# lambdaclass/noir_backend_using_gnark

Hardware: AMD Instinct MI355X
Metric: Groth16 prove ms + BN254 G1 MSM scalar-muls/sec at 2^20 / 2^24 constraints (higher is better)
Workload: dtype u32; 1 GPU; groth16_prove_bn254_synthetic_r1cs_2^20; constraints=1048576, wires=1048576, n_public=8, scalars=uniform, per_gpu_constraints=1048576, window_tables=True, parallelism=single GPU

## Files before the change

include/zkmi.h:

```cpp
#ifndef ZKMI_H
#define ZKMI_H
#include <stddef.h>
#include <stdint.h>
#ifdef __cplusplus
extern "C" {
#endif

typedef struct { uint64_t l[4]; } zk_fr;
typedef struct { uint64_t l[4]; } zk_fp;
typedef struct { zk_fp x, y; } zk_g1_affine;
typedef struct { zk_fp x0, x1, y0, y1; } zk_g2_affine;

typedef enum {
    ZK_OK = 0,
    ZK_ERR_LEN = -1,
    ZK_ERR_NB_TASKS = -2,
    ZK_ERR_NO_DEVICE = -3,
    ZK_ERR_HIP = -4,
    ZK_ERR_ARG = -5,
    ZK_ERR_HANDLE = -6,
    ZK_ERR_BUSY = -7
} zk_status;

typedef struct {
// ... 155 lines not shown
        const void *const *vks, const size_t *vk_lens, size_t n_keys, int vk_is_hex,
        const zk_g2_affine srs_g2[2], const uint32_t *key_of ,
        const zk_fr *public_inputs, size_t pub_stride,
        uint8_t *accepted, size_t *n_accepted);
int zk_bn254_plonk_verify_batch_keys_dev(const void *d_proofs, size_t proof_stride, size_t n_proofs,
        const void *const *vks, const size_t *vk_lens, size_t n_keys, int vk_is_hex,
        const zk_g2_affine srs_g2[2], const uint32_t *key_of ,
        const void *d_public_inputs, size_t pub_stride,
        uint8_t *accepted, size_t *n_accepted);

int zk_bn254_groth16_msm5_dev(const void *d_a, const void *d_b, const void *d_b2, const void *d_w, size_t nw,
                              const void *d_k, const void *d_wk, size_t nk, const void *d_z, const void *d_h, size_t nz,
                              uint64_t out_xyzz[96], void *stream);
int zk_bn254_groth16_msm5_pk(uint64_t pk_handle, const void *d_w, const void *d_h, uint64_t out_xyzz[96], void *stream);
int zk_bn254_groth16_msm5_pk_begin(uint64_t pk_handle, const void *d_w, uint64_t *session);
int zk_bn254_groth16_msm5_pk_end(uint64_t session, const void *d_h, uint64_t out_xyzz[96], void *stream);
int zk_bn254_groth16_msm5_pk_abort(uint64_t session);
int zk_bn254_groth16_msm5_session_stream(uint64_t session, void **stream_out);
int zk_bn254_groth16_finalize(uint64_t pk_handle, const uint64_t *partials, size_t n_partials, const zk_fr *r,
                              const zk_fr *s, uint8_t proof_out[128]);
int zk_bn254_groth16_finalize_batch(uint64_t pk_handle, const uint64_t *partials, size_t n_partials, const zk_fr *r, const zk_fr *s,
                                    size_t n_proofs, uint8_t *proofs_out);
int zk_bn254_groth16_finalize_batch_dev(uint64_t pk_handle, const void *d_partials, size_t n_partials, const void *d_r, const void *d_s,
                                        size_t n_proofs, void *d_proofs_out, void *stream);

typedef struct {
    size_t n_public, n_constraints, n_vars;
    const void *ql, *qr, *qo, *qm, *qk;
    const uint32_t *xa, *xb, *xc;
    int coeffs_on_device;
    int reserved;
} zk_plonk_circuit;
typedef struct {
    uint32_t log_n;
    size_t n_public, n_constraints, n_vars;
    const zk_fr *ql, *qr, *qm, *qo, *cqk, *lqk, *s1, *s2, *s3;
    const int64_t *permutation;
    const uint32_t *xa, *xb, *xc;
    const zk_g1_affine *vk_s , *vk_ql, *vk_qr, *vk_qm, *vk_qo, *vk_qk;
} zk_plonk_pk;
typedef struct {
    uint64_t size, n_public;
    zk_fr size_inv, generator, coset_shift;
    zk_g1_affine s[3], ql, qr, qm, qo, qk;
} zk_plonk_vk;
int zk_bn254_plonk_setup(const zk_plonk_circuit *circuit, uint64_t srs_handle, uint64_t *pk_handle, zk_plonk_vk *vk_out);
int zk_bn254_plonk_pk_load(const zk_plonk_pk *pk, uint64_t srs_handle, uint64_t *pk_handle);
int zk_bn254_plonk_pk_free(uint64_t pk_handle);
int zk_bn254_plonk_pk_lagrange_srs(uint64_t pk_handle);
int zk_bn254_plonk_pk_read(const void *data, size_t len, int is_hex, size_t n_vars, size_t n_constraints, const uint32_t *xa,
                           const uint32_t *xb, const uint32_t *xc, uint64_t srs_handle, uint64_t *pk_handle);
int zk_bn254_plonk_pk_write(uint64_t pk_handle, int as_hex, void *out, size_t cap, size_t *out_len);
int zk_bn254_plonk_pk_info(uint64_t pk_handle, size_t *domain_size, size_t *n_public, size_t *n_constraints, size_t *n_vars);
int zk_bn254_plonk_pk_export(uint64_t pk_handle, int which, zk_fr *out_host, size_t n);
enum { ZK_PLONK_PROOF_BYTES = 548 };
int zk_bn254_plonk_prove(uint64_t pk_handle, const void *solution, size_t n_vars, int on_device, const zk_fr blinders[9],
                         const zk_fr *challenges, uint8_t proof_out[ZK_PLONK_PROOF_BYTES]);
int zk_bn254_plonk_synth_qk_dev(void *d_qk, const void *d_ql, const void *d_qr, const void *d_qo, const void *d_qm, const void *d_xa,
                                const void *d_xb, const void *d_xc, const void *d_solution, size_t n_constraints, void *stream);

int zk_bn254_iop_sigma_dev(const void *d_perm, uint32_t log_n, void *d_sigma, void *stream);
int zk_bn254_iop_ratio_copy_batch_dev(const void *d_l, const void *d_r, const void *d_o, size_t in_stride, uint32_t log_n, size_t rows, const void *d_sigma,
                                      const void *d_beta, const void *d_gamma, void *d_z, size_t out_stride, void *stream);
int zk_bn254_iop_ratio_copy_batch(const zk_fr *l, const zk_fr *r, const zk_fr *o, uint32_t log_n, size_t rows, const uint32_t *perm, const zk_fr *beta,
                                  const zk_fr *gamma, zk_fr *z_out);
int zk_bn254_plonk_ratio_batch_dev(uint64_t pk_handle, const void *d_l, const void *d_r, const void *d_o, size_t in_stride, size_t rows, const void *d_beta,
                                   const void *d_gamma, void *d_z, size_t out_stride, void *stream);
int zk_bn254_fr_batch_invert_dev(void *d_a, size_t n, void *stream);

int zk_bn254_plonk_quotient_batch_dev(uint64_t pk_handle, const void *d_l, const void *d_r, const void *d_o, const void *d_z, size_t in_stride, const void *d_pub,
                                      size_t pub_stride, size_t rows, const void *d_alpha, const void *d_beta, const void *d_gamma, void *d_h, size_t out_stride,
                                      void *d_status, void *stream);

int zk_bn254_fr_poly_open_rows_dev(const void *d_f, size_t in_stride, size_t len, size_t rows, const void *d_points, void *d_q, size_t q_stride, void *d_values,
                                   void *stream);
int zk_bn254_plonk_linearize_batch_dev(uint64_t pk_handle, const void *d_l, const void *d_r, const void *d_o, const void *d_z, size_t in_stride, const void *d_h,
                                       size_t h_stride, size_t rows, const void *d_alpha, const void *d_beta, const void *d_gamma, const void *d_zeta, void *d_values,
                                       void *d_zquot, void *d_lin, void *d_fh, size_t out_stride, void *stream);
int zk_bn254_plonk_open_batch_dev(uint64_t pk_handle, const void *d_fh, const void *d_lin, const void *d_l, const void *d_r, const void *d_o, size_t in_stride,
                                  size_t rows, const void *d_zeta, const void *d_kzg_gamma, void *d_q, size_t out_stride, void *d_value, void *stream);
int zk_bn254_plonk_commit_batch_dev(uint64_t pk_handle, const void *d_rows, size_t row_stride, size_t len, size_t rows, int from_values, void *d_out,
                                    void *d_compressed);

int zk_bn254_plonk_prove_batch(uint64_t pk_handle, const void *solutions, size_t n_vars, size_t sol_stride, size_t rows, int on_device,
                               const zk_fr *blinders , const zk_fr *challenges , size_t chunk_rows ,
                               uint8_t *proofs_out , int *status_out );
int zk_bn254_plonk_prove_batch_info(uint64_t pk_handle, size_t *chunk_rows, int *commits_batched, int *lin_by_linearity);
int zk_bn254_plonk_challenges_batch_dev(uint64_t pk_handle, int stage, size_t rows, const void *d_pub, size_t pub_stride, const void *d_points,
                                        const void *d_prev, const void *d_values, void *d_out, void *stream);

enum { ZK_ACIR_LAYOUT_REFERENCE = 0, ZK_ACIR_LAYOUT_ONE_VAR_PER_WITNESS = 1 };
int zk_plonk_preprocess(const char *acir_json, size_t acir_len, const char *values_hex, size_t values_len, int layout,
                        uint64_t srs_handle, char *pk_hex_out, size_t pk_cap, size_t *pk_len, char *vk_hex_out, size_t vk_cap,
                        size_t *vk_len, uint64_t *pk_handle);
int zk_plonk_prove_with_pk(const char *acir_json, size_t acir_len, const char *values_hex, size_t values_len, int layout,
                           const char *pk_hex, size_t pk_len, uint64_t pk_handle, uint64_t srs_handle, const zk_fr *blinders,
                           char proof_hex_out[2 * ZK_PLONK_PROOF_BYTES]);
int zk_acir_to_sparse_r1cs(const char *acir_json, size_t acir_len, size_t n_values, int layout, size_t *n_public, size_t *n_vars,
                           size_t *n_constraints, zk_fr *ql, zk_fr *qr, zk_fr *qo, zk_fr *qm, zk_fr *qk, uint32_t *xa, uint32_t *xb,
                           uint32_t *xc, uint32_t *order);
int zk_acir_public_witnesses(const char *acir_json, size_t acir_len, size_t n_values, int layout, uint32_t *out, size_t cap, size_t *n_public);
int zk_export_cache_info(size_t *n_circuits, size_t *n_keys, size_t *bytes);
int zk_acir_lower_resident(const char *acir_json, size_t acir_len, size_t n_values, int layout, int with_coefficients);
int zk_export_cache_clear(void);
int zk_export_set_new_srs_size(size_t n);
size_t zk_export_new_srs_size(void);
int zk_bn254_plonk_pk_bytes(uint64_t handle, size_t *bytes);

int zk_groth16_r1cs_from_raw(const char *raw_json, size_t len, uint64_t *r1cs_handle, void **d_witness, size_t *n_wires, size_t *n_public);
int zk_groth16_preprocess(const char *raw_json, size_t raw_len, const zk_fr *toxic, char *pk_hex_out, size_t pk_cap, size_t *pk_len,
                          char *vk_hex_out, size_t vk_cap, size_t *vk_len, uint64_t *pk_handle);
int zk_groth16_prove_with_pk(const char *raw_json, size_t raw_len, const char *pk_hex, size_t pk_len, uint64_t pk_handle, const zk_fr *rs,
                             char proof_hex_out[256]);
int zk_groth16_prove_with_meta(const char *raw_json, size_t raw_len, const zk_fr *toxic, const zk_fr *rs, char proof_hex_out[256]);
int zk_groth16_lower_resident(const char *raw_json, size_t raw_len, int to_device);
int zk_groth16_key_resident(const char *pk_hex, size_t pk_len);
int zk_groth16_public_inputs(const char *raw_json, size_t raw_len, zk_fr *out, size_t cap, size_t *n_public);

enum {
    ZK_ROW_OK = 0,
    ZK_ROW_UNSATISFIED = 1,
    ZK_ROW_BAD_HEX = 2,
    ZK_ROW_NOT_CANONICAL = 3,
    ZK_ROW_BAD_COUNT = 4,
    ZK_ROW_BAD_PROOF_HEX
};
int zk_plonk_solutions_rows(const char *acir_json, size_t acir_len, int layout, const char *values_hex, size_t values_len, size_t values_stride,
                            size_t rows, void *d_solutions , size_t sol_stride, int *status_out );
int zk_groth16_wires_rows(const char *raw_json, size_t raw_len, const char *values_hex, size_t values_len, size_t values_stride,
                          size_t rows, void *d_wires , size_t wire_stride, int *status_out );
int zk_plonk_prove_batch_with_pk(const char *acir_json, size_t acir_len, int layout, const char *values_hex, size_t values_len, size_t values_stride,
                                 size_t rows, const char *pk_hex, size_t pk_len, uint64_t pk_handle, uint64_t srs_handle,
                                 const zk_fr *blinders , size_t chunk_rows ,
                                 char *proofs_hex_out , int *status_out );
int zk_groth16_prove_batch_with_pk(const char *raw_json, size_t raw_len, const char *values_hex, size_t values_len, size_t values_stride, size_t rows,
                                   const char *pk_hex, size_t pk_len, uint64_t pk_handle, const zk_fr *rs ,
                                   size_t chunk_rows, char *proofs_hex_out , int *status_out );

int zk_plonk_verify_batch_with_vk(const char *acir_json, size_t acir_len, int layout, const char *proofs_hex, size_t proofs_stride,
                                  const char *values_hex, size_t values_len, size_t values_stride, size_t rows, const char *vk_hex, size_t vk_len,
                                  const zk_g2_affine srs_g2[2], size_t chunk_rows, uint8_t *accepted , int *status_out ,
                                  size_t *n_accepted);
int zk_groth16_verify_batch_with_vk(const char *raw_json, size_t raw_len, const char *proofs_hex, size_t proofs_stride, const char *values_hex,
                                    size_t values_len, size_t values_stride, size_t rows, const char *vk_hex, size_t vk_len, size_t chunk_rows,
                                    uint8_t *accepted , int *status_out , size_t *n_accepted);

int zk_bn254_msm_plan_info(size_t n, int window_tables, uint32_t *window_bits, uint32_t *digits);

typedef struct {
    size_t n;
    int window_bits, scalars_mont, table, drop_zero_digits;
    uint32_t c, row_first, row_step, sets;
    size_t stride;
    int by_rows, reserved;
    const zk_fr *vec[3];
    size_t row_stride;
} zk_msm_prep_request;
typedef struct {
    uint32_t c, W, Wd, Wrows, B, nb, key_bits, L, Lmin, m1, N1, dropped;
    uint64_t total, max_tasks, device_total;
    uint32_t ctl[64];
    uint32_t *keys, *vals, *start, *task_off, *task_begin, *len_keys, *task_ids, *multi_list;
} zk_msm_prep_result;
int zk_bn254_msm_prep_inspect(const zk_msm_prep_request *req, zk_msm_prep_result *res);

#define ZK_MSM_TAIL_MAX_LEVELS 12
typedef struct {
    zk_msm_prep_request prep;
    const void *points;
    int is_g2, quad_tail, keep_final, reserved;
    uint32_t l1_m, l2_m, skip_below, reserved2;
} zk_msm_tail_request;
typedef struct {
    uint32_t kind, n_in, n_out, sh_in, sh_out, m;
} zk_msm_tail_level;
typedef struct {
    zk_msm_prep_result prep;
    uint32_t m2, tasks, n_final, sh_final, n_levels, reserved;
    zk_msm_tail_level level[ZK_MSM_TAIL_MAX_LEVELS];
    uint64_t table_entries, level_entries;
    uint64_t *table, *partial_acc, *partial_fold, *level_a, *level_s, *set_values, *total, *final_affine;
    uint8_t *final_bytes;
} zk_msm_tail_result;
int zk_bn254_msm_tail_inspect(const zk_msm_tail_request *req, zk_msm_tail_result *res);

#define ZK_HSCAN_ROWS_MAX 8
typedef struct {
    uint32_t rows, K, nb, pad;
    int eval_only, reserved;
    zk_fr *f[ZK_HSCAN_ROWS_MAX], *q[ZK_HSCAN_ROWS_MAX];
    size_t len[ZK_HSCAN_ROWS_MAX];
    zk_fr a[ZK_HSCAN_ROWS_MAX];
} zk_hscan_request;
typedef struct {
    uint32_t nb, reserved;
    zk_fr *tcarry, *btot_local, *btot, *total;
} zk_hscan_result;
int zk_bn254_hscan_inspect(const zk_hscan_request *req, zk_hscan_result *res);

int zk_bn254_felts_decode_hex(const char *hex, size_t hex_len, void *d_out, size_t cap, size_t *n_out);
int zk_bn254_felts_decode_hex_dev(const void *d_text, size_t text_len, void *d_out, size_t cap, size_t n, int to_mont,
                                  void *stream);
int zk_bn254_felts_decode_bytes_dev(const void *d_raw, size_t raw_len, void *d_out, size_t cap, size_t n, int to_mont,
                                    void *stream);
int zk_bn254_felts_encode_hex(const void *d_in, size_t n, char *hex_out, size_t cap);
int zk_bn254_felts_decode_hex_rows_dev(const void *d_text, size_t pitch, size_t rows, size_t n, void *d_out, size_t out_stride,
                                       int to_mont, int *d_status , void *stream);
int zk_bn254_bytes_decode_hex_rows_dev(const void *d_text, size_t pitch, size_t rows, size_t n_bytes, void *d_out, size_t out_stride,
                                       int *d_status , void *stream);
int zk_bn254_felts_public_hex_rows_dev(const void *d_text, size_t pitch, size_t rows, size_t n_values, const uint32_t *d_where, size_t n_public,
                                       void *d_pub, size_t pub_stride, int *d_status , void *stream);

int zk_bn254_fr_random_dev(void *d_out, size_t n, uint64_t seed, int mont, int witness_like, void *stream);
int zk_bn254_g1_generate_dev(void *d_out, size_t n, uint64_t seed, void *stream);
int zk_bn254_g2_generate_dev(void *d_out, size_t n, uint64_t seed, void *stream);
int zk_bn254_fr_mul_dev(void *d_out, const void *d_a, const void *d_b, size_t n, void *stream);

int zk_bn254_kzg_new_srs_dev(void *d_g1_out, size_t size, const zk_fr *alpha, zk_g2_affine g2_out[2], void *stream);
int zk_bn254_kzg_srs_read(const void *data, size_t len, int is_hex, int table_window_bits, uint64_t *handle, size_t *n_g1,
                          zk_g2_affine g2_out[2]);
int zk_bn254_kzg_srs_write(uint64_t handle, const zk_g2_affine g2[2], int as_hex, void *out, size_t cap, size_t *out_len);
int zk_bn254_kzg_srs_g2(const void *data, size_t len, int is_hex, zk_g2_affine g2_out[2]);

typedef struct { zk_g1_affine h; zk_fr claimed_value; } zk_kzg_opening;
int zk_bn254_kzg_open(uint64_t srs, const void *const *polys, const size_t *lens, const zk_fr *points, size_t count, int on_device, zk_kzg_opening *out);
int zk_bn254_kzg_batch_open_single_point(uint64_t srs, const void *const *polys, const size_t *lens, const zk_g1_affine *digests, size_t count,
                                         const zk_fr *point, int on_device, zk_g1_affine *out_h, zk_fr *out_claimed);
int zk_bn254_kzg_verify(const zk_g1_affine *digest, const zk_kzg_opening *opening, const zk_fr *point, const zk_g2_affine srs_g2[2], int *accepted);
int zk_bn254_kzg_fold_proof(const zk_g1_affine *digests, size_t count, const zk_g1_affine *h, const zk_fr *claimed, const zk_fr *point,
                            zk_kzg_opening *out_opening, zk_g1_affine *out_digest);
int zk_bn254_kzg_batch_verify_single_point(const zk_g1_affine *digests, size_t count, const zk_g1_affine *h, const zk_fr *claimed, const zk_fr *point,
                                           const zk_g2_affine srs_g2[2], int *accepted);
int zk_bn254_kzg_verify_batch(const zk_g1_affine *digests, const zk_kzg_opening *openings, const zk_fr *points, size_t n_openings,
                              const zk_g2_affine srs_g2[2], uint8_t *accepted, size_t *n_accepted);

int zk_dev_alloc(void **d_ptr, size_t bytes);
int zk_dev_free(void *d_ptr);
int zk_dev_h2d(void *d_dst, const void *h_src, size_t bytes);
int zk_dev_d2h(void *h_dst, const void *d_src, size_t bytes);
int zk_dev_sync(void);

int zk_profile_enable(int on);
int zk_profile_host(const char *name, double ms);
int zk_profile_reset(void);
int zk_profile_count(void);
int zk_profile_get(int idx, char *name_out, size_t name_cap, uint64_t *launches, double *total_ms);

int zk_selftest_host(void);

#ifdef __cplusplus
}
#endif
#endif
```

noir_backend_using_gnark_amd/_lib.py:

```python
from __future__ import annotations

import ctypes as C
import os

_HERE = os.path.dirname(os.path.abspath(__file__))
LIB_PATH = os.path.join(_HERE, "libzkmi.so")


def use_library(path: str) -> None:
    global LIB_PATH, _lib
    if _lib is not None:
        raise RuntimeError("the library is already loaded from %s" % LIB_PATH)
    LIB_PATH = path


ZK_OK, ZK_ERR_LEN, ZK_ERR_NB_TASKS, ZK_ERR_NO_DEVICE, ZK_ERR_HIP, ZK_ERR_ARG, ZK_ERR_HANDLE, ZK_ERR_BUSY = 0, -1, -2, -3, -4, -5, -6, -7


class ZkmiError(RuntimeError):
    def __init__(self, code: int, msg: str):
        super().__init__("libzkmi error %d: %s" % (code, msg))
        self.code = code


class MsmCfg(C.Structure):
    _fields_ = [("nb_tasks", C.c_int), ("scalars_mont", C.c_int), ("window_bits", C.c_int), ("device_mask", C.c_int)]


class MsmPrepRequest(C.Structure):
    _fields_ = [("n", C.c_size_t), ("window_bits", C.c_int), ("scalars_mont", C.c_int), ("table", C.c_int), ("drop_zero_digits", C.c_int),
                ("c", C.c_uint32), ("row_first", C.c_uint32), ("row_step", C.c_uint32), ("sets", C.c_uint32), ("stride", C.c_size_t),
                ("by_rows", C.c_int), ("reserved", C.c_int), ("vec", C.c_void_p * 3), ("row_stride", C.c_size_t)]


MSM_PREP_PLAN = ("c", "W", "Wd", "Wrows", "B", "nb", "key_bits", "L", "Lmin", "m1", "N1")
MSM_PREP_ARRAYS = ("keys", "vals", "start", "task_off", "task_begin", "len_keys", "task_ids", "multi_list")


class MsmPrepResult(C.Structure):
    _fields_ = [(k, C.c_uint32) for k in MSM_PREP_PLAN + ("dropped",)] + [("total", C.c_uint64), ("max_tasks", C.c_uint64), ("device_total", C.c_uint64),
                                                                         ("ctl", C.c_uint32 * 64)] + [(k, C.c_void_p) for k in MSM_PREP_ARRAYS]


MSM_TAIL_MAX_LEVELS = 12
MSM_TAIL_LEVEL = ("kind", "n_in", "n_out", "sh_in", "sh_out", "m")
MSM_TAIL_KINDS = {1: "l1", 2: "l2", 3: "wave", 4: "wave_quad"}
MSM_TAIL_ARRAYS = ("table", "partial_acc", "partial_fold", "level_a", "level_s", "set_values", "total", "final_affine", "final_bytes")


class MsmTailRequest(C.Structure):
    _fields_ = [("prep", MsmPrepRequest), ("points", C.c_void_p), ("is_g2", C.c_int), ("quad_tail", C.c_int), ("keep_final", C.c_int), ("reserved", C.c_int),
                ("l1_m", C.c_uint32), ("l2_m", C.c_uint32), ("skip_below", C.c_uint32), ("reserved2", C.c_uint32)]


class MsmTailLevel(C.Structure):
    _fields_ = [(k, C.c_uint32) for k in MSM_TAIL_LEVEL]


class MsmTailResult(C.Structure):
    _fields_ = [("prep", MsmPrepResult)] + [(k, C.c_uint32) for k in ("m2", "tasks", "n_final", "sh_final", "n_levels", "reserved")] + \
               [("level", MsmTailLevel * MSM_TAIL_MAX_LEVELS), ("table_entries", C.c_uint64), ("level_entries", C.c_uint64)] + \
               [(k, C.c_void_p) for k in MSM_TAIL_ARRAYS]


HSCAN_ROWS_MAX = 8


class HscanRequest(C.Structure):
    _fields_ = [("rows", C.c_uint32), ("K", C.c_uint32), ("nb", C.c_uint32), ("pad", C.c_uint32), ("eval_only", C.c_int), ("reserved", C.c_int),
                ("f", C.c_void_p * HSCAN_ROWS_MAX), ("q", C.c_void_p * HSCAN_ROWS_MAX), ("len", C.c_size_t * HSCAN_ROWS_MAX),
                ("a", (C.c_uint64 * 4) * HSCAN_ROWS_MAX)]


class HscanResult(C.Structure):
    _fields_ = [("nb", C.c_uint32), ("reserved", C.c_uint32)] + [(k, C.c_void_p) for k in ("tcarry", "btot_local", "btot", "total")]


class Groth16PK(C.Structure):
    _fields_ = [("log_domain", C.c_uint32), ("n_wires", C.c_size_t), ("n_public", C.c_size_t),
                ("g1_alpha", C.c_void_p), ("g1_beta", C.c_void_p), ("g1_delta", C.c_void_p),
                ("g1_a", C.c_void_p), ("g1_b", C.c_void_p), ("g1_k", C.c_void_p), ("g1_z", C.c_void_p),
                ("g2_beta", C.c_void_p), ("g2_delta", C.c_void_p), ("g2_b", C.c_void_p), ("bases_on_device", C.c_int), ("flags", C.c_int),
                ("infinity_a", C.c_void_p), ("infinity_b", C.c_void_p), ("nb_infinity_a", C.c_size_t), ("nb_infinity_b", C.c_size_t),
                ("table_window_bits", C.c_int), ("device_mask", C.c_int), ("shard_rank", C.c_uint32), ("shard_count", C.c_uint32)]


class R1CS(C.Structure):
    _fields_ = [("n_constraints", C.c_size_t), ("n_wires", C.c_size_t), ("n_public", C.c_size_t)] + \
               [(m + k, C.c_void_p) for m in ("l", "r", "o") for k in ("_ptr", "_idx", "_val")]


class PlonkCircuit(C.Structure):
    _fields_ = [("n_public", C.c_size_t), ("n_constraints", C.c_size_t), ("n_vars", C.c_size_t),
                ("ql", C.c_void_p), ("qr", C.c_void_p), ("qo", C.c_void_p), ("qm", C.c_void_p), ("qk", C.c_void_p),
                ("xa", C.c_void_p), ("xb", C.c_void_p), ("xc", C.c_void_p), ("coeffs_on_device", C.c_int), ("reserved", C.c_int)]


class PlonkPK(C.Structure):
    _fields_ = [("log_n", C.c_uint32), ("n_public", C.c_size_t), ("n_constraints", C.c_size_t), ("n_vars", C.c_size_t)] + \
               [(k, C.c_void_p) for k in ("ql", "qr", "qm", "qo", "cqk", "lqk", "s1", "s2", "s3", "permutation", "xa", "xb", "xc",
                                          "vk_s", "vk_ql", "vk_qr", "vk_qm", "vk_qo", "vk_qk")]


class PlonkVK(C.Structure):
    _fields_ = [("size", C.c_uint64), ("n_public", C.c_uint64), ("size_inv", C.c_uint64 * 4), ("generator", C.c_uint64 * 4), ("coset_shift", C.c_uint64 * 4),
                ("s", C.c_uint64 * 24), ("ql", C.c_uint64 * 8), ("qr", C.c_uint64 * 8), ("qm", C.c_uint64 * 8), ("qo", C.c_uint64 * 8), ("qk", C.c_uint64 * 8)]


PLONK_PROOF_BYTES = 548

SYMBOLS = [
    "zk_device_count", "zk_init", "zk_last_error", "zk_version",
    "zk_bn254_g1_msm", "zk_bn254_g2_msm", "zk_bn254_g1_msm_dev", "zk_bn254_g2_msm_dev",
    "zk_bn254_g1_msm_partial_dev", "zk_bn254_g2_msm_partial_dev", "zk_bn254_g1_sum_xyzz", "zk_bn254_g2_sum_xyzz",
    "zk_bn254_msm_plan_info", "zk_bn254_msm_prep_inspect", "zk_bn254_msm_tail_inspect", "zk_bn254_bases_register", "zk_bn254_bases_register_dev", "zk_bn254_bases_register_cfg", "zk_bn254_bases_build_table", "zk_bn254_bases_lagrange", "zk_bn254_bases_free", "zk_bn254_msm_bases", "zk_bn254_msm_bases_batch", "zk_bn254_msm_bases_batch_dev", "zk_bn254_msm_bases_dev", "zk_bn254_scalars_register", "zk_bn254_scalars_free", "zk_bn254_msm_bases_prepared",
    "zk_bn254_ntt", "zk_bn254_ntt_dev", "zk_bn254_bit_reverse", "zk_bn254_bit_reverse_dev",
    "zk_bn254_ntt_batch", "zk_bn254_ntt_batch_dev", "zk_bn254_groth16_compute_h_batch", "zk_bn254_groth16_compute_h_batch_dev",
    "zk_bn254_groth16_compute_h", "zk_bn254_groth16_compute_h_dev", "zk_bn254_groth16_h_shard_dev", "zk_bn254_ntt_shard_dev",
    "zk_bn254_felts_decode_hex", "zk_bn254_felts_decode_hex_dev", "zk_bn254_felts_decode_bytes_dev", "zk_bn254_felts_encode_hex",
    "zk_bn254_groth16_pk_load", "zk_bn254_groth16_pk_free", "zk_bn254_groth16_pk_info", "zk_bn254_groth16_prove",
    "zk_bn254_groth16_pk_read", "zk_bn254_groth16_pk_write", "zk_bn254_groth16_vk_write",
    "zk_bn254_groth16_verify", "zk_bn254_plonk_verify", "zk_bn254_pairing_check",
    "zk_bn254_pair", "zk_bn254_pair_host", "zk_bn254_groth16_verify_batch", "zk_bn254_plonk_verify_batch",
    "zk_bn254_r1cs_load", "zk_bn254_r1cs_free", "zk_bn254_r1cs_eval_abc_dev", "zk_bn254_r1cs_eval_abc_rows_dev", "zk_bn254_groth16_setup", "zk_bn254_groth16_prove_r1cs",
    "zk_bn254_groth16_prove_batch", "zk_bn254_groth16_prove_r1cs_batch", "zk_bn254_groth16_batch_info",
    "zk_bn254_groth16_msm5_dev", "zk_bn254_groth16_msm5_pk", "zk_bn254_groth16_msm5_pk_begin", "zk_bn254_groth16_msm5_pk_end", "zk_bn254_groth16_msm5_pk_abort", "zk_bn254_groth16_msm5_session_stream", "zk_bn254_groth16_finalize",
    "zk_bn254_groth16_finalize_batch", "zk_bn254_groth16_finalize_batch_dev",
    "zk_bn254_plonk_setup", "zk_bn254_plonk_pk_load", "zk_bn254_plonk_pk_free", "zk_bn254_plonk_pk_lagrange_srs", "zk_bn254_plonk_pk_export", "zk_bn254_plonk_pk_read", "zk_bn254_plonk_pk_write", "zk_bn254_plonk_prove", "zk_bn254_plonk_synth_qk_dev",
    "zk_bn254_iop_sigma_dev", "zk_bn254_iop_ratio_copy_batch_dev", "zk_bn254_iop_ratio_copy_batch", "zk_bn254_plonk_ratio_batch_dev", "zk_bn254_fr_batch_invert_dev", "zk_bn254_plonk_quotient_batch_dev",
    "zk_bn254_fr_poly_open_rows_dev", "zk_bn254_plonk_linearize_batch_dev", "zk_bn254_plonk_open_batch_dev",
    "zk_plonk_preprocess", "zk_plonk_prove_with_pk", "zk_bn254_plonk_pk_info", "zk_acir_to_sparse_r1cs", "zk_groth16_r1cs_from_raw",
    "zk_groth16_preprocess", "zk_groth16_prove_with_pk", "zk_groth16_prove_with_meta",
    "zk_bn254_fr_random_dev", "zk_bn254_g1_generate_dev", "zk_bn254_g2_generate_dev", "zk_bn254_fr_mul_dev", "zk_bn254_kzg_new_srs_dev", "zk_bn254_kzg_srs_read", "zk_bn254_kzg_srs_write",
    "zk_dev_alloc", "zk_dev_free", "zk_dev_h2d", "zk_dev_d2h", "zk_dev_sync",
    "zk_profile_enable", "zk_profile_reset", "zk_profile_count", "zk_profile_get", "zk_profile_host", "zk_selftest_host",
    "zk_init_devices", "zk_warm_streams", "zk_init_flags", "zk_bn254_kzg_srs_g2", "zk_device_entries", "zk_set_entry", "zk_set_default_devices", "zk_default_devices", "zk_bn254_ntt_devices",
    "zk_acir_public_witnesses", "zk_acir_lower_resident", "zk_export_cache_info", "zk_export_cache_clear", "zk_bn254_plonk_pk_bytes",
    "zk_groth16_lower_resident", "zk_groth16_key_resident", "zk_groth16_public_inputs", "zk_bn254_groth16_pk_build_tables", "zk_bn254_groth16_pk_bytes",
    "zk_export_set_new_srs_size", "zk_export_new_srs_size", "zk_warm_session_streams", "zk_warm_session_streams_background", "zk_background_wait", "zk_background_hold", "zk_background_set_yield_ms", "zk_bn254_bases_build_table_background",
    "zk_bn254_msm_bases_rows", "zk_bn254_msm_bases_rows_dev", "zk_bn254_msm_rows_info", "zk_bn254_plonk_commit_batch_dev",
    "zk_bn254_plonk_prove_batch", "zk_bn254_plonk_prove_batch_info", "zk_bn254_plonk_challenges_batch_dev",
    "zk_bn254_felts_decode_hex_rows_dev", "zk_plonk_solutions_rows", "zk_groth16_wires_rows", "zk_plonk_prove_batch_with_pk", "zk_groth16_prove_batch_with_pk",
    "zk_bn254_groth16_verify_batch_dev", "zk_bn254_plonk_verify_batch_dev", "zk_bn254_rows_sha256_dev", "zk_bn254_bytes_decode_hex_rows_dev",
    "zk_bn254_felts_public_hex_rows_dev", "zk_plonk_verify_batch_with_vk", "zk_groth16_verify_batch_with_vk",
    "zk_bn254_kzg_open", "zk_bn254_kzg_batch_open_single_point", "zk_bn254_kzg_verify", "zk_bn254_kzg_fold_proof", "zk_bn254_kzg_batch_verify_single_point", "zk_bn254_kzg_verify_batch",
    "zk_bn254_plonk_verify_batch_keys", "zk_bn254_plonk_verify_batch_keys_dev",
    "zk_bn254_hscan_inspect",
]

_SZ, _VP, _CP = C.c_size_t, C.c_void_p, C.c_char_p
ARGTYPES = {
    "zk_bn254_felts_decode_hex_rows_dev": [_VP, _SZ, _SZ, _SZ, _VP, _SZ, C.c_int, _VP, _VP],
    "zk_plonk_solutions_rows": [_CP, _SZ, C.c_int, _CP, _SZ, _SZ, _SZ, _VP, _SZ, _VP],
    "zk_groth16_wires_rows": [_CP, _SZ, _CP, _SZ, _SZ, _SZ, _VP, _SZ, _VP],
    "zk_plonk_prove_batch_with_pk": [_CP, _SZ, C.c_int, _CP, _SZ, _SZ, _SZ, _CP, _SZ, C.c_uint64, C.c_uint64, _VP, _SZ, _VP, _VP],
    "zk_groth16_prove_batch_with_pk": [_CP, _SZ, _CP, _SZ, _SZ, _SZ, _CP, _SZ, C.c_uint64, _VP, _SZ, _VP, _VP],
    "zk_bn254_groth16_verify_batch_dev": [_VP, _SZ, _SZ, _CP, _SZ, C.c_int, _VP, _SZ, _SZ, _VP, _VP],
    "zk_bn254_plonk_verify_batch_dev": [_VP, _SZ, _SZ, _CP, _SZ, C.c_int, _VP, _VP, _SZ, _SZ, _VP, _VP],
    "zk_bn254_rows_sha256_dev": [_VP, _SZ, _SZ, _VP, _SZ, _SZ, _SZ, _VP, _VP],
    "zk_bn254_bytes_decode_hex_rows_dev": [_VP, _SZ, _SZ, _SZ, _VP, _SZ, _VP, _VP],
    "zk_bn254_felts_public_hex_rows_dev": [_VP, _SZ, _SZ, _SZ, _VP, _SZ, _VP, _SZ, _VP, _VP],
    "zk_plonk_verify_batch_with_vk": [_CP, _SZ, C.c_int, _CP, _SZ, _CP, _SZ, _SZ, _SZ, _CP, _SZ, _VP, _SZ, _VP, _VP, _VP],
    "zk_groth16_verify_batch_with_vk": [_CP, _SZ, _CP, _SZ, _CP, _SZ, _SZ, _SZ, _CP, _SZ, _SZ, _VP, _VP, _VP],
    "zk_bn254_plonk_verify_batch_keys": [_VP, _SZ, _VP, _VP, _SZ, C.c_int, _VP, _VP, _VP, _SZ, _VP, _VP],
    "zk_bn254_plonk_verify_batch_keys_dev": [_VP, _SZ, _SZ, _VP, _VP, _SZ, C.c_int, _VP, _VP, _VP, _SZ, _VP, _VP],
}
ROW_OK, ROW_UNSATISFIED, ROW_BAD_HEX, ROW_NOT_CANONICAL, ROW_BAD_COUNT, ROW_BAD_PROOF_HEX = 0, 1, 2, 3, 4, 5

_lib = None


def lib() -> C.CDLL:
    global _lib
    if _lib is None:
        if not os.path.exists(LIB_PATH):
            raise RuntimeError(
                "libzkmi.so is missing at %s: build it with `python -c 'import __graft_entry__ as g; g.build()'` "
                "(make -C noir_backend_using_gnark_amd/csrc).  There is no CPU fallback for the product path." % LIB_PATH)
        _lib = C.CDLL(LIB_PATH)
        _lib.zk_last_error.restype = C.c_char_p
        _lib.zk_version.restype = C.c_char_p
        for name in SYMBOLS:
            fn = getattr(_lib, name)
            if name == "zk_export_new_srs_size":
                fn.restype = C.c_size_t
            elif name not in ("zk_last_error", "zk_version"):
                fn.restype = C.c_int
            if name in ARGTYPES:
                fn.argtypes = ARGTYPES[name]
    return _lib


def check(rc: int) -> None:
    if rc != ZK_OK:
# ... 81 lines not shown
```

noir_backend_using_gnark_amd/bn254.py:

```python
from __future__ import annotations

import ctypes as C
from dataclasses import dataclass

import numpy as np

from . import _lib
from ._lib import MsmCfg, check, lib, vp

DIT, DIF = 0, 1


@dataclass
class MultiExpConfig:
    nb_tasks: int = 0
    scalars_mont: bool = False
    window_bits: int = 0
    device_mask: int = 0

    def _c(self) -> MsmCfg:
        return MsmCfg(self.nb_tasks, 1 if self.scalars_mont else 0, self.window_bits, self.device_mask)


def _as_u64(a, width) -> np.ndarray:
    a = np.ascontiguousarray(a, dtype=np.uint64)
    if a.size % width:
        raise ValueError("array size %d is not a multiple of %d limbs" % (a.size, width))
    return a.reshape(-1, width)


def _multi_exp(fn, width, points, scalars, config):
    config = config or MultiExpConfig()
    points, scalars = _as_u64(points, width), _as_u64(scalars, 4)
    if points.shape[0] != scalars.shape[0]:
        pass
    out = np.zeros(width, dtype=np.uint64)
    cfg = config._c()
    rc = fn(vp(points), C.c_size_t(points.shape[0]), vp(scalars), C.c_size_t(scalars.shape[0]), C.byref(cfg), vp(out))
    if rc in (_lib.ZK_ERR_LEN, _lib.ZK_ERR_NB_TASKS):
        raise ValueError((lib().zk_last_error() or b"").decode())
    check(rc)
    return out


def g1_multi_exp(points, scalars, config: MultiExpConfig | None = None) -> np.ndarray:
    return _multi_exp(lib().zk_bn254_g1_msm, 8, points, scalars, config)


def g2_multi_exp(points, scalars, config: MultiExpConfig | None = None) -> np.ndarray:
    return _multi_exp(lib().zk_bn254_g2_msm, 16, points, scalars, config)


def g1_multi_exp_dev(d_points: int, d_scalars: int, n: int, config: MultiExpConfig | None = None, stream: int = 0, partial=False):
    cfg = (config or MultiExpConfig())._c()
    out = np.zeros(16 if partial else 8, dtype=np.uint64)
    fn = lib().zk_bn254_g1_msm_partial_dev if partial else lib().zk_bn254_g1_msm_dev
    check(fn(C.c_void_p(d_points), C.c_void_p(d_scalars), C.c_size_t(n), C.byref(cfg), vp(out), C.c_void_p(stream)))
    return out


def g2_multi_exp_dev(d_points: int, d_scalars: int, n: int, config: MultiExpConfig | None = None, stream: int = 0, partial=False):
    cfg = (config or MultiExpConfig())._c()
    out = np.zeros(32 if partial else 16, dtype=np.uint64)
    fn = lib().zk_bn254_g2_msm_partial_dev if partial else lib().zk_bn254_g2_msm_dev
    check(fn(C.c_void_p(d_points), C.c_void_p(d_scalars), C.c_size_t(n), C.byref(cfg), vp(out), C.c_void_p(stream)))
    return out


def g1_sum_partials(partials) -> np.ndarray:
    p = _as_u64(partials, 16)
    out = np.zeros(8, dtype=np.uint64)
    check(lib().zk_bn254_g1_sum_xyzz(vp(p), C.c_size_t(p.shape[0]), vp(out)))
    return out


def g2_sum_partials(partials) -> np.ndarray:
    p = _as_u64(partials, 32)
    out = np.zeros(16, dtype=np.uint64)
    check(lib().zk_bn254_g2_sum_xyzz(vp(p), C.c_size_t(p.shape[0]), vp(out)))
    return out


def _msm_prep_request(req, vectors, n, window_bits, scalars_mont, table_c, stride, row_first, row_step, rows, row_stride, drop_zero_digits):
    if rows:
        mat = _as_u64(vectors, 4)
        row_stride = row_stride if row_stride is not None else mat.shape[0] // rows
        if n is None:
            n = row_stride
        if mat.shape[0] < (rows - 1) * row_stride + n:
            raise ValueError("the matrix is shorter than rows * row_stride")
        keep, sets = [mat], rows
    else:
        keep, seen = [], {}
        for v in (vectors if isinstance(vectors, (list, tuple)) else [vectors]):
            if id(v) not in seen:
                seen[id(v)] = _as_u64(v, 4)
            keep.append(seen[id(v)])
        sets = len(keep)
        if n is None:
            n = keep[0].shape[0]
        if any(k.shape[0] < n for k in keep):
            raise ValueError("a scalar vector is shorter than n")
    req.n, req.window_bits, req.scalars_mont, req.table, req.drop_zero_digits = n, window_bits, int(scalars_mont), int(table_c != 0), int(drop_zero_digits)
    req.c, req.row_first, req.row_step, req.sets, req.stride = table_c, row_first, row_step, sets, (stride if stride is not None else n)
    req.by_rows, req.row_stride = int(rows > 0), (row_stride or 0)
    for i, k in enumerate(keep[:3]):
        req.vec[i] = k.ctypes.data
    return keep


def _msm_prep_plan(res) -> dict:
    return dict({k: int(getattr(res, k)) for k in _lib.MSM_PREP_PLAN}, total=int(res.total), max_tasks=int(res.max_tasks))


def _msm_prep_arrays(res, plan, arrays) -> dict:
    sizes = dict(keys=plan["total"], vals=plan["total"], start=plan["nb"] + 1, task_off=plan["nb"] + 1, task_begin=plan["max_tasks"], len_keys=plan["max_tasks"],
                 task_ids=plan["max_tasks"], multi_list=plan["nb"])
    wanted = _lib.MSM_PREP_ARRAYS if arrays is None else tuple(arrays)
    out = {k: np.zeros(sizes[k] if k in wanted else 0, np.uint32) for k in _lib.MSM_PREP_ARRAYS}
    for k in wanted:
        setattr(res, k, out[k].ctypes.data)
    return out


def msm_prep_inspect(vectors, n: int | None = None, window_bits: int = 0, scalars_mont: bool = False, table_c: int = 0, stride: int | None = None,
                     row_first: int = 0, row_step: int = 1, rows: int = 0, row_stride: int | None = None, drop_zero_digits: bool = False,
                     plan_only: bool = False, arrays=None) -> dict:
    req = _lib.MsmPrepRequest()
    keep = _msm_prep_request(req, vectors, n, window_bits, scalars_mont, table_c, stride, row_first, row_step, rows, row_stride, drop_zero_digits)
    res = _lib.MsmPrepResult()
    check(lib().zk_bn254_msm_prep_inspect(C.byref(req), C.byref(res)))
    out = _msm_prep_plan(res)
    if plan_only or out["total"] == 0:
        out.update(device_total=0, dropped=False, ctl=np.zeros(64, np.uint32), **{k: np.zeros(0, np.uint32) for k in _lib.MSM_PREP_ARRAYS})
        return out
    arrays = _msm_prep_arrays(res, out, arrays)
    check(lib().zk_bn254_msm_prep_inspect(C.byref(req), C.byref(res)))
    assert _msm_prep_plan(res) == out
    out.update(device_total=int(res.device_total), dropped=bool(res.dropped), ctl=np.array(res.ctl[:], dtype=np.uint32), **arrays)
    return out


def msm_tail_inspect(points, vectors, is_g2: bool = False, l1_m: int = 0, l2_m: int = 0, quad_tail: bool = False, keep_final: bool = False, skip_below: int = 0,
                     plan_only: bool = False, **prep) -> dict:
    width = 16 if is_g2 else 8
    pts = _as_u64(points, width)
    req = _lib.MsmTailRequest()
    keep = _msm_prep_request(req.prep, vectors, prep.pop("n", None), prep.pop("window_bits", 0), prep.pop("scalars_mont", False), prep.pop("table_c", 0),
                             prep.pop("stride", None), prep.pop("row_first", 0), prep.pop("row_step", 1), prep.pop("rows", 0), prep.pop("row_stride", None),
                             prep.pop("drop_zero_digits", False))
    if prep:
        raise TypeError("unknown arguments: %s" % sorted(prep))
    if pts.shape[0] < req.prep.n:
        raise ValueError("fewer points than scalars")
    req.points, req.is_g2, req.quad_tail, req.keep_final = pts.ctypes.data, int(is_g2), int(quad_tail), int(keep_final)
    req.l1_m, req.l2_m, req.skip_below = l1_m, l2_m, skip_below
    res = _lib.MsmTailResult()
    check(lib().zk_bn254_msm_tail_inspect(C.byref(req), C.byref(res)))

    def plan():
        d = _msm_prep_plan(res.prep)
        d.update({k: int(getattr(res, k)) for k in ("m2", "n_final", "sh_final", "table_entries", "level_entries")})
        d["levels"] = [dict({k: int(getattr(res.level[i], k)) for k in _lib.MSM_TAIL_LEVEL}, kind=_lib.MSM_TAIL_KINDS[int(res.level[i].kind)])
                       for i in range(res.n_levels)]
        return d
    out = plan()
    sets = int(req.prep.sets) if req.prep.table else 1
    if plan_only or (out["total"] == 0 and not keep_final):
        return out
    arrays = _msm_prep_arrays(res.prep, out, None) if out["total"] else {}
    W = out["W"]
    shapes = dict(table=(out["table_entries"], width), partial_acc=(out["max_tasks"], width), partial_fold=(out["max_tasks"], width),
                  level_a=(out["level_entries"], width), level_s=(out["level_entries"], width))
    if keep_final:
        shapes.update(final_affine=(sets, 8), final_bytes=(sets, 32))
    else:
        shapes.update(set_values=(W, width), total=(1, width))
    tail = {k: np.zeros(shp, np.uint8 if k == "final_bytes" else np.uint64) for k, shp in shapes.items()}
    for k, a in tail.items():
        setattr(res, k, a.ctypes.data)
    check(lib().zk_bn254_msm_tail_inspect(C.byref(req), C.byref(res)))
    assert plan() == out
    if out["total"]:
        out.update(device_total=int(res.prep.device_total), dropped=bool(res.prep.dropped), ctl=np.array(res.prep.ctl[:], dtype=np.uint32), **arrays)
    out["tasks"] = int(res.tasks)
    at = 0
    for lv in out["levels"]:
        cnt = W * lv["n_out"]
        lv["A"] = tail["level_a"][at:at + cnt].reshape(W, lv["n_out"], width)
        lv["S"] = tail["level_s"][at:at + cnt].reshape(W, lv["n_out"], width)
        at += cnt
    out.update({k: v for k, v in tail.items() if k not in ("level_a", "level_s")})
    return out


MSM_ROWS_SPARSE, MSM_ROWS_NO_POINTS = 1, 2
_DEV = (int, _lib.DeviceBuffer)


def _dptr(a) -> int:
    return a if isinstance(a, int) else a.ptr


def _check_len(rc: int) -> None:
    if rc in (_lib.ZK_ERR_LEN, _lib.ZK_ERR_NB_TASKS):
        raise ValueError((lib().zk_last_error() or b"").decode())
    check(rc)


def rows_digests(dev_call, host_call, scalars, n, rows, row_stride, out, compressed, points):
    if not isinstance(compressed, bool) and not isinstance(compressed, _DEV):
        raise TypeError("compressed must be False, True or a device buffer / pointer")
    if not points and compressed is False:
        raise ValueError("points=False leaves nothing to return: ask for the compressed digests")
    if not points and out is not None:
        raise ValueError("out takes the points: there are none with points=False")
    if isinstance(scalars, _DEV):
        if n is None or rows is None:
            raise ValueError("n and rows are required with device-resident scalars")
        n, rows = int(n), int(rows)
        if n < 0 or rows < 0:
            raise ValueError("n and rows must not be negative")
        row_stride = int(n if row_stride is None else row_stride)
        if row_stride < n and rows > 1:
            raise ValueError("row_stride = %d is below the n = %d scalars of a row" % (row_stride, n))
        span = ((rows - 1) * row_stride + n) * 32 if rows and n else 0
        if isinstance(scalars, _lib.DeviceBuffer) and span > scalars.nbytes:
            raise ValueError("scalars: %d bytes do not fit the device buffer (%d bytes)" % (span, scalars.nbytes))
        seen = [("scalars", scalars, span)]
        for name, b, nbytes in (("out", out, rows * 64), ("compressed", compressed, rows * 32)):
            if b is None or isinstance(b, bool):
                continue
            if not isinstance(b, _DEV):
                raise TypeError("%s must be a device buffer or a device pointer" % name)
            if isinstance(b, _lib.DeviceBuffer) and nbytes > b.nbytes:
                raise ValueError("%s: %d bytes do not fit the device buffer (%d bytes)" % (name, nbytes, b.nbytes))
            for other, c, cb in seen:
                if nbytes and cb and _dptr(b) < _dptr(c) + cb and _dptr(c) < _dptr(b) + nbytes:
                    raise ValueError("%s overlaps %s" % (name, other))
            seen.append((name, b, nbytes))
        made = []
        if points and out is None:
            out = _lib.DeviceBuffer(max(rows * 64, 64))
            made.append(out)
        if compressed is True:
            compressed = _lib.DeviceBuffer(max(rows * 32, 32))
            made.append(compressed)
        enc = None if compressed is False else compressed
        if rows:
            try:
                _check_len(dev_call(_dptr(scalars), row_stride, n, rows, _dptr(out) if points else 0, _dptr(enc) if enc is not None else 0))
            except Exception:
                for b in made:
                    b.free()
                raise
        return out if enc is None else ((out, enc) if points else enc)
    if not (isinstance(scalars, np.ndarray) and scalars.dtype == np.uint64 and scalars.flags["C_CONTIGUOUS"]):
        raise TypeError("scalars must be a C-contiguous uint64 numpy array (or a device buffer)")
    if scalars.ndim != 3 or scalars.shape[2] != 4:
        raise ValueError("scalars has shape %s, not (rows, n, 4)" % (scalars.shape,))
    cnt, width = scalars.shape[0], scalars.shape[1]
    for name, v, want in (("rows", rows, cnt), ("n", n, width), ("row_stride", row_stride, width)):
        if v is not None and int(v) != want:
            raise ValueError("%s = %d != %d of the host array (its rows are contiguous)" % (name, v, want))
    if out is not None or not isinstance(compressed, bool):
        raise ValueError("out and a compressed buffer belong to the device form: the host form returns new arrays")
    pts = np.zeros((cnt, 8), np.uint64) if points else None
    enc = np.zeros((cnt, 32), np.uint8) if compressed else None
    if cnt and host_call is not None:
        _check_len(host_call(scalars, width, cnt, pts, enc))
    elif cnt:
        bufs = [_lib.DeviceBuffer.from_numpy(scalars), _lib.DeviceBuffer(cnt * 64), _lib.DeviceBuffer(cnt * 32)]
        try:
            _check_len(dev_call(bufs[0].ptr, width, width, cnt, bufs[1].ptr if points else 0, bufs[2].ptr if compressed else 0))
            pts = bufs[1].to_numpy(np.uint64, (cnt, 8)) if points else None
            enc = bufs[2].to_numpy(np.uint8, (cnt, 32)) if compressed else None
        finally:
            for b in bufs:
                b.free()
    return pts if enc is None else ((pts, enc) if points else enc)


def msm_rows_info(bases: "ResidentBases", n: int, sparse: bool = False) -> dict:
    chunk, batched = C.c_size_t(0), C.c_int(0)
    _check_len(lib().zk_bn254_msm_rows_info(bases.handle, C.c_size_t(n), C.c_uint32(MSM_ROWS_SPARSE if sparse else 0), C.byref(chunk), C.byref(batched)))
    return {"chunk_rows": int(chunk.value), "batched": bool(batched.value)}


class ResidentBases:

    def __init__(self, points, is_g2: bool = False, n: int | None = None, table_window_bits: int = 0):
        self.is_g2, self.handle = is_g2, C.c_uint64(0)
        if isinstance(points, (_lib.DeviceBuffer, int)):
            if n is None:
                raise ValueError("n is required with device-resident points")
            self.n = n
            ptr = points.ptr if isinstance(points, _lib.DeviceBuffer) else int(points)
            check(lib().zk_bn254_bases_register_cfg(C.c_void_p(ptr), C.c_size_t(n), C.c_int(int(is_g2)), C.c_int(1), C.c_int(table_window_bits), C.byref(self.handle)))
            return
        points = _as_u64(points, 16 if is_g2 else 8)
        self.n = points.shape[0]
        check(lib().zk_bn254_bases_register_cfg(vp(points), C.c_size_t(self.n), C.c_int(int(is_g2)), C.c_int(0), C.c_int(table_window_bits), C.byref(self.handle)))

    def multi_exp_dev(self, d_scalars, n: int, config: MultiExpConfig | None = None, offset: int = 0) -> np.ndarray:
        out = np.zeros(16 if self.is_g2 else 8, dtype=np.uint64)
        cfg = (config or MultiExpConfig())._c()
        ptr = d_scalars.ptr if isinstance(d_scalars, _lib.DeviceBuffer) else int(d_scalars)
        rc = lib().zk_bn254_msm_bases_dev(self.handle, C.c_size_t(offset), C.c_void_p(ptr), C.c_size_t(n), C.byref(cfg), vp(out))
        if rc in (_lib.ZK_ERR_LEN, _lib.ZK_ERR_NB_TASKS):
            raise ValueError((lib().zk_last_error() or b"").decode())
        check(rc)
        return out

    def multi_exp(self, scalars, config: MultiExpConfig | None = None, offset: int = 0) -> np.ndarray:
# ... 213 lines not shown
```

noir_backend_using_gnark_amd/csrc/msm.hip:

```cpp
#include <math.h>
#include <string.h>

#include <algorithm>
#include <memory>
#include <tuple>
#include <type_traits>

#ifdef ZKMI_EXPERIMENTS
#include "experiments/msm_rocprim_include.inc"
#endif

#include <chrono>
#include "codec_dev.hpp"
#include "ctx.hpp"
#include "curve.hpp"
#include "ff29.hpp"
#include "host_ff.hpp"
#include "msm.hpp"
#include "multidev.hpp"
#include "proofio.hpp"
#include "radix.hpp"

namespace zkmi {

struct PingPong {
    uint32_t* b[2];
    int cur = 0;
    PingPong(uint32_t* x, uint32_t* y) : b{x, y} {}
    uint32_t* current() const { return b[cur]; }
    uint32_t* alternate() const { return b[cur ^ 1]; }
    void swap() { cur ^= 1; }
};
#ifdef ZKMI_EXPERIMENTS
#include "experiments/msm_rocprim_config.inc"
#endif

static int rs_sort_pairs(Slot* s, hipStream_t st, void* tmp, PingPong& kb, PingPong& vb, size_t n, unsigned key_bits, const uint32_t* d_n = nullptr) {
    const RsPlan R = rs_plan(n, key_bits);
    uint32_t* tile_hist = (uint32_t*)tmp;
    uint32_t* ghist = tile_hist + (size_t)RS_MAX_BINS * R.ntiles;
    uint32_t* gbase = ghist + RS_MAX_PASSES * RS_MAX_BINS;
    RsArgs A;
    A.npass = R.npass;
    for (unsigned p = 0; p < RS_MAX_PASSES; p++) { A.shift[p] = R.shift[p]; A.bits[p] = R.bits[p]; }
    const unsigned nt = (unsigned)R.ntiles;
    ZK_HIP(hipMemsetAsync(ghist, 0, RS_MAX_PASSES * RS_MAX_BINS * 4, st));
    ZK_LAUNCH(s, st, "msm_sort_hist", k_rs_hist, dim3(nt), dim3(RS_THREADS), 0, (const uint32_t*)kb.current(), (uint32_t)n, A, nt, ghist, tile_hist, d_n);
    ZK_LAUNCH(s, st, "msm_sort_bases", k_rs_bases, dim3(1), dim3(RS_MAX_BINS), 0, (const uint32_t*)ghist, gbase, R.npass);
    for (unsigned p = 0; p < R.npass; p++) {
        if (p) ZK_LAUNCH(s, st, "msm_sort_hist", k_rs_tile_hist, dim3(nt), dim3(RS_THREADS), 0, (const uint32_t*)kb.current(), (uint32_t)n, R.shift[p], R.bits[p], nt, tile_hist, d_n);
        ZK_LAUNCH(s, st, "msm_sort_scan", k_rs_scan_rows, dim3(1u << R.bits[p]), dim3(256), 0, tile_hist, nt);
        ZK_LAUNCH(s, st, "msm_sort_pass", k_rs_scatter, dim3(nt), dim3(RS_THREADS), 0, (const uint32_t*)kb.current(), (const uint32_t*)vb.current(), kb.alternate(), vb.alternate(),
                  (uint32_t)n, R.shift[p], R.bits[p], nt, (const uint32_t*)tile_hist, (const uint32_t*)(gbase + p * RS_MAX_BINS), d_n);
        kb.swap();
        vb.swap();
    }
    return ZK_OK;
}

static int xs_exclusive_scan(Slot* s, hipStream_t st, void* tmp, const uint32_t* in, uint32_t* out, size_t n) {
    const unsigned nt = (unsigned)((n + XS_TILE - 1) / XS_TILE);
    uint32_t* sums = (uint32_t*)tmp;
    ZK_LAUNCH(s, st, "msm_task_scan", k_xs_sums, dim3(nt), dim3(XS_THREADS), 0, in, (uint32_t)n, sums);
    ZK_LAUNCH(s, st, "msm_task_scan", k_xs_scan_sums, dim3(1), dim3(XS_THREADS), 0, sums, nt);
    ZK_LAUNCH(s, st, "msm_task_scan", k_xs_apply, dim3(nt), dim3(XS_THREADS), 0, in, (uint32_t)n, (const uint32_t*)sums, out);
    return ZK_OK;
}

template <class T>
__device__ __forceinline__ T gload(const T* p) {
    static_assert(sizeof(T) % 16 == 0, "16-byte multiples only");
    T r;
    const uint4* q = reinterpret_cast<const uint4*>(p);
    uint4* d = reinterpret_cast<uint4*>(&r);
#pragma unroll
    for (unsigned i = 0; i < sizeof(T) / 16; i++) d[i] = q[i];
    return r;
}
template <class T>
__device__ __forceinline__ void gstore(T* p, const T& v) {
    uint4* q = reinterpret_cast<uint4*>(p);
    const uint4* d = reinterpret_cast<const uint4*>(&v);
#pragma unroll
    for (unsigned i = 0; i < sizeof(T) / 16; i++) q[i] = d[i];
}
template <class T>
__device__ __forceinline__ T shfl_down_t(const T& v, unsigned d) {
    T r;
    const uint32_t* s = reinterpret_cast<const uint32_t*>(&v);
    uint32_t* o = reinterpret_cast<uint32_t*>(&r);
#pragma unroll
    for (unsigned i = 0; i < sizeof(T) / 4; i++) o[i] = __shfl_down(s[i], d, 64);
    return r;
}
template <class T>
__device__ __forceinline__ T shfl_xor_t(const T& v, unsigned d) {
    T r;
    const uint32_t* s = reinterpret_cast<const uint32_t*>(&v);
    uint32_t* o = reinterpret_cast<uint32_t*>(&r);
#pragma unroll
    for (unsigned i = 0; i < sizeof(T) / 4; i++) o[i] = __shfl_xor(s[i], d, 64);
    return r;
}

struct DigitSrc {
    const Fr* p[3];
    __device__ __forceinline__ const Fr* vec(unsigned v) const { return p[v]; }
};
struct DigitRows {
    const Fr* base;
    size_t stride;
    __device__ __forceinline__ const Fr* vec(unsigned v) const { return base + (size_t)v * stride; }
};
template <class Src>
__global__ void k_msm_digits(Src src, uint32_t n, int mont, unsigned c, unsigned W, uint32_t* keys, uint32_t* vals,
                             uint32_t table_stride, unsigned row_first, unsigned row_step, unsigned rows_per_set) {
    prio_hi();
    uint32_t i = blockIdx.x * blockDim.x + threadIdx.x;
    if (i >= n) return;
    const unsigned vec = blockIdx.y, sets = gridDim.y;
    const Fr* scalars = src.vec(vec);
    Fr s;
    {
        const uint4* q = reinterpret_cast<const uint4*>(scalars + i);
        uint4 a = q[0], b = q[1];
        s.l[0] = a.x; s.l[1] = a.y; s.l[2] = a.z; s.l[3] = a.w;
        s.l[4] = b.x; s.l[5] = b.y; s.l[6] = b.z; s.l[7] = b.w;
    }
    if (mont) s = s.from_mont();
    const uint32_t B = 1u << (c - 1);
    const uint32_t sentinel = table_stride ? sets * B : W * B;
    uint32_t carry = 0;
    unsigned next_row = row_first, wl = 0;
    for (unsigned w = 0; w < W; w++) {
        unsigned bit = w * c, limb = bit >> 5, off = bit & 31;
        uint64_t v = 0;
        if (limb < 8) {
            v = s.l[limb];
            if (limb + 1 < 8) v |= (uint64_t)s.l[limb + 1] << 32;
            v >>= off;
        }
        uint32_t d = ((uint32_t)v & ((1u << c) - 1)) + carry;
        carry = 0;
        uint32_t neg = 0, mag = d;
        if (d > B) {
            mag = (1u << c) - d;
            neg = 1;
            carry = 1;
        }
        size_t o = (size_t)w * n + i;
        if (table_stride) {
            if (w != next_row) continue;
            o = ((size_t)vec * rows_per_set + wl) * n + i;
            keys[o] = mag ? (vec * B + (mag - 1)) : sentinel;
            vals[o] = ((wl * table_stride + i) << 1) | neg;
            next_row += row_step;
            wl++;
        } else {
            keys[o] = mag ? (w * B + (mag - 1)) : sentinel;
            vals[o] = (i << 1) | neg;
        }
    }
}

__device__ __forceinline__ Fr canonical_scalar(const Fr* __restrict__ scalars, uint32_t i, int mont) {
    Fr s;
    const uint4* q = reinterpret_cast<const uint4*>(scalars + i);
    uint4 a = q[0], b = q[1];
    s.l[0] = a.x; s.l[1] = a.y; s.l[2] = a.z; s.l[3] = a.w;
    s.l[4] = b.x; s.l[5] = b.y; s.l[6] = b.z; s.l[7] = b.w;
    return mont ? s.from_mont() : s;
}
template <class Emit>
__device__ __forceinline__ void digits_of(const Fr& s, unsigned c, unsigned W, bool table, unsigned row_first, unsigned row_step, Emit&& emit) {
    const uint32_t B = 1u << (c - 1);
    uint32_t carry = 0;
    unsigned next_row = row_first, wl = 0;
    for (unsigned w = 0; w < W; w++) {
        unsigned bit = w * c, limb = bit >> 5, off = bit & 31;
        uint64_t v = 0;
        if (limb < 8) {
            v = s.l[limb];
            if (limb + 1 < 8) v |= (uint64_t)s.l[limb + 1] << 32;
            v >>= off;
        }
        uint32_t d = ((uint32_t)v & ((1u << c) - 1)) + carry;
        carry = 0;
        uint32_t neg = 0, mag = d;
        if (d > B) {
            mag = (1u << c) - d;
            neg = 1;
            carry = 1;
        }
        if (!table) { emit(w, mag, neg); continue; }
        if (w != next_row) continue;
        emit(wl, mag, neg);
        next_row += row_step;
        wl++;
    }
}
template <class Src>
__global__ __launch_bounds__(256) void k_msm_digits_compact(Src src, uint32_t n, int mont, unsigned c, unsigned W, unsigned row_first, unsigned row_step,
                                                           uint32_t table_stride, uint32_t* __restrict__ total, uint32_t* __restrict__ keys, uint32_t* __restrict__ vals) {
    prio_hi();
    extern __shared__ uint32_t stage[];
    __shared__ uint32_t wsum[4];
    __shared__ uint32_t base;
    const uint32_t i = blockIdx.x * blockDim.x + threadIdx.x;
    const unsigned vec = blockIdx.y;
    const uint32_t B = 1u << (c - 1), cap = 256u * W;
    const bool live = i < n;
    uint32_t k = 0;
    Fr sc = Fr::zero();
    if (live) {
        sc = canonical_scalar(src.vec(vec), i, mont);
        digits_of(sc, c, W, table_stride != 0, row_first, row_step, [&](unsigned, uint32_t mag, uint32_t) { k += mag != 0; });
    }
    uint32_t incl = k;
    const unsigned lane = threadIdx.x & 63, wave = threadIdx.x >> 6;
#pragma unroll
    for (int d = 1; d < 64; d <<= 1) {
        const uint32_t up = (uint32_t)__shfl_up((int)incl, d, 64);
        if (lane >= (unsigned)d) incl += up;
    }
    if (lane == 63) wsum[wave] = incl;
    __syncthreads();
    uint32_t before = 0;
    for (unsigned w2 = 0; w2 < wave; w2++) before += wsum[w2];
    const uint32_t wg_total = wsum[0] + wsum[1] + wsum[2] + wsum[3];
    if (threadIdx.x == 0) base = wg_total ? atomicAdd(total, wg_total) : 0;
    if (live && k) {
        uint32_t o = before + incl - k;
        digits_of(sc, c, W, table_stride != 0, row_first, row_step, [&](unsigned wl, uint32_t mag, uint32_t neg) {
            if (!mag) return;
            if (table_stride) {
                stage[o] = vec * B + (mag - 1);
                stage[cap + o] = ((wl * table_stride + i) << 1) | neg;
            } else {
                stage[o] = wl * B + (mag - 1);
                stage[cap + o] = (i << 1) | neg;
            }
            o++;
        });
    }
    __syncthreads();
    const uint32_t g0 = base;
    for (uint32_t j = threadIdx.x; j < wg_total; j += 256) {
        keys[g0 + j] = stage[j];
        vals[g0 + j] = stage[cap + j];
    }
}

__global__ void k_bucket_bounds(const uint32_t* __restrict__ keys, uint32_t total, uint32_t nb, uint32_t* __restrict__ start, const uint32_t* __restrict__ d_total) {
    prio_hi();
    uint32_t b = blockIdx.x * blockDim.x + threadIdx.x;
    if (b > nb) return;
    total = rs_len(total, d_total);
    uint32_t lo = 0, hi = total;
    while (lo < hi) {
        uint32_t mid = lo + ((hi - lo) >> 1);
        if (keys[mid] < b) lo = mid + 1; else hi = mid;
    }
    start[b] = lo;
}

constexpr uint32_t GIANT_T = 256;
constexpr uint32_t GIANT_MAX = 48;
constexpr uint32_t GIANT_POINTS = 8192;
__device__ __forceinline__ uint32_t giant_seg(uint32_t cnt) {
    const uint32_t s = ((cnt + 63) / 64 + 63) / 64 * 64;
    return s < 64 ? 64 : s;
}
__global__ __launch_bounds__(256) void k_bucket_stats(const uint32_t* __restrict__ start, uint32_t nb, uint32_t* __restrict__ ctl) {
    prio_hi();
    __shared__ uint32_t wmax[4];
    uint32_t len = 0;
    uint32_t big = 0;
    for (uint32_t b = blockIdx.x * blockDim.x + threadIdx.x; b < nb; b += gridDim.x * blockDim.x) {
        const uint32_t l = start[b + 1] - start[b];
        len = max(len, l);
        big += l > GIANT_POINTS ? 1u : 0u;
    }
    if (big) atomicAdd(&ctl[3], big);
    for (int d = 32; d > 0; d >>= 1) len = max(len, (uint32_t)__shfl_down((int)len, d, 64));
    if ((threadIdx.x & 63) == 0) wmax[threadIdx.x >> 6] = len;
    __syncthreads();
    if (threadIdx.x == 0) {
        len = max(max(wmax[0], wmax[1]), max(wmax[2], wmax[3]));
        if (len) atomicMax(&ctl[1], len);
    }
}
__global__ void k_pick_len(const uint32_t* __restrict__ start, uint32_t nb, uint32_t Lmax, uint32_t Lmin, uint32_t lanes, uint32_t factor, uint32_t cap,
                           uint32_t flat_keeps, uint32_t* __restrict__ ctl) {
    prio_hi();
    const uint32_t nnz = start[nb], biggest = ctl[1];
    const uint32_t q = (nnz + lanes - 1) / lanes;
    uint32_t lw = factor * q;
    if (2 * lw < Lmax) lw = (factor / 2 ? factor / 2 : 1) * q;
    if (ctl[3] > GIANT_MAX) cap = cap > 2048 ? 2048 : cap;
    uint32_t lg = (biggest + cap - 1) / cap;
    uint32_t L = max(max(lw, lg), Lmin);
    if (flat_keeps && biggest <= Lmax && nb * 8 >= lanes) L = Lmax;
    ctl[2] = min(L, Lmax);
}
__global__ void k_task_plan(const uint32_t* start, uint32_t nb, const uint32_t* __restrict__ ctl, uint32_t* ntasks, uint32_t* multi_list, uint32_t* num_multi) {
    prio_hi();
    uint32_t b = blockIdx.x * blockDim.x + threadIdx.x;
    if (b > nb) return;
    if (b == nb) { ntasks[b] = 0; return; }
    const uint32_t L = ctl[2];
    uint32_t cnt = start[b + 1] - start[b];
    uint32_t t = (cnt + L - 1) / L;
    ntasks[b] = t;
    if (t > 1) multi_list[atomicAdd(num_multi, 1u)] = b;
    if (t > GIANT_T) {
        const uint32_t gi = atomicAdd(&num_multi[4], 1u);
        if (gi < GIANT_MAX) num_multi[8 + gi] = b;
    }
}

__device__ __forceinline__ bool block_arrive_is_last(uint32_t* counter, uint32_t expected) {
    __shared__ uint32_t is_last;
    __threadfence();
    asm volatile("s_waitcnt vmcnt(0)" ::: "memory");
    __syncthreads();
    if (threadIdx.x == 0) {
        __threadfence();
        asm volatile("s_waitcnt vmcnt(0)" ::: "memory");
        is_last = (atomicAdd(counter, 1u) + 1 == expected) ? 1u : 0u;
    }
    __syncthreads();
    if (!is_last) return false;
    __threadfence();
    asm volatile("s_waitcnt vmcnt(0)" ::: "memory");
    return true;
}

__global__ __launch_bounds__(256) void k_bucket_stats_pick(const uint32_t* __restrict__ start, uint32_t nb, uint32_t Lmax, uint32_t Lmin, uint32_t lanes, uint32_t factor,
                                                           uint32_t cap, uint32_t flat_keeps, uint32_t* __restrict__ ctl) {
    prio_hi();
    __shared__ uint32_t wmax[4];
    uint32_t len = 0;
    uint32_t big = 0;
    for (uint32_t b = blockIdx.x * blockDim.x + threadIdx.x; b < nb; b += gridDim.x * blockDim.x) {
        const uint32_t l = start[b + 1] - start[b];
        len = max(len, l);
        big += l > GIANT_POINTS ? 1u : 0u;
    }
    if (big) atomicAdd(&ctl[3], big);
    for (int d = 32; d > 0; d >>= 1) len = max(len, (uint32_t)__shfl_down((int)len, d, 64));
    if ((threadIdx.x & 63) == 0) wmax[threadIdx.x >> 6] = len;
    __syncthreads();
    if (threadIdx.x == 0) {
        len = max(max(wmax[0], wmax[1]), max(wmax[2], wmax[3]));
        if (len) atomicMax(&ctl[1], len);
    }
    if (!block_arrive_is_last(&ctl[5], gridDim.x)) return;
    if (threadIdx.x == 0) {
        const uint32_t nnz = start[nb], biggest = atomicAdd(&ctl[1], 0u), nbig = atomicAdd(&ctl[3], 0u);
        const uint32_t q = (nnz + lanes - 1) / lanes;
        uint32_t lw = factor * q;
        if (2 * lw < Lmax) lw = (factor / 2 ? factor / 2 : 1) * q;
        if (nbig > GIANT_MAX) cap = cap > 2048 ? 2048 : cap;
        const uint32_t lg = (biggest + cap - 1) / cap;
        uint32_t L = max(max(lw, lg), Lmin);
        if (flat_keeps && biggest <= Lmax && nb * 8 >= lanes) L = Lmax;
        ctl[2] = min(L, Lmax);
    }
// ... 332 lines not shown
    unsigned first = 32;
    while (first >= cnt && first > 0) first >>= 1;
    for (unsigned d = first; d > 0; d >>= 1) {
        TailPt<F> o = acc.shfl_down(d);
        if (lane < d) acc.add(o);
    }
    if (lane == 0) acc.store(partial + lo);
}
template <class F>
__global__ __launch_bounds__(256) void k_fold_multi(XYZZ<F>* partial, const uint32_t* task_off, const uint32_t* multi_list,
                                                    const uint32_t* num_multi) {
    prio_hi();
    const uint32_t lane = threadIdx.x & 63, wave = threadIdx.x >> 6;
    const uint32_t nm = *num_multi;
    for (uint32_t m = blockIdx.x * 4 + wave; m < nm; m += gridDim.x * 4) {
        uint32_t b = multi_list[m];
        uint32_t t0 = task_off[b], t1 = task_off[b + 1];
        TailPt<F> acc = TailPt<F>::inf();
        uint32_t nheld = t1 - t0;
        bool listed = false;
        if (nheld > GIANT_T) {
            const uint32_t ng = min(num_multi[4], GIANT_MAX);
            listed = __ballot(lane < ng && num_multi[8 + lane] == b) != 0;
        }
        if (listed) {
            const uint32_t S = giant_seg(nheld);
            nheld = (nheld + S - 1) / S;
            if (lane < nheld) acc = TailPt<F>::load(partial + t0 + lane * S);
        } else {
            for (uint32_t t = t0 + lane; t < t1; t += 64) acc.add(TailPt<F>::load(partial + t));
        }
        const uint32_t cnt = min(nheld, 64u);
        unsigned first = 32;
        while (first >= cnt && first > 0) first >>= 1;
        for (unsigned d = first; d > 0; d >>= 1) {
            TailPt<F> o = acc.shfl_down(d);
            if (lane < d) acc.add(o);
        }
        if (lane == 0) acc.store(partial + t0);
    }
}

template <class F, class PT = TailPt<F>>
__global__ __launch_bounds__(256) void k_reduce_l1(const XYZZ<F>* __restrict__ partial, const uint32_t* __restrict__ task_off, uint32_t B,
                                                   uint32_t W, uint32_t m, XYZZ<F>* __restrict__ A_out, XYZZ<F>* __restrict__ S_out) {
    prio_hi();
    uint32_t N1 = B / m;
    uint32_t g = (blockIdx.x * blockDim.x + threadIdx.x) / PT::LPP;
    if (g >= W * N1) return;
    uint32_t w = g / N1, q = g % N1;
    uint32_t b0 = w * B + q * m;
    PT run = PT::inf(), acc = PT::inf();
    for (int l = (int)m - 1; l >= 0; l--) {
        uint32_t b = b0 + l;
        uint32_t t0 = task_off[b];
        if (task_off[b + 1] > t0) run.add(PT::load(partial + t0));
        acc.add(run);
    }
    if (threadIdx.x % PT::LPP == 0) {
        acc.store(A_out + g);
        run.store(S_out + g);
    }
}

template <class F>
__global__ __launch_bounds__(256) void k_reduce_l2(const XYZZ<F>* __restrict__ A_in, const XYZZ<F>* __restrict__ S_in, uint32_t N, uint32_t W, uint32_t sh,
                                                   uint32_t m, XYZZ<F>* __restrict__ A_out, XYZZ<F>* __restrict__ S_out) {
    prio_hi();
    typedef TailPt<F> PT;
    uint32_t Nout = (N + m - 1) / m;
    uint32_t g = blockIdx.x * blockDim.x + threadIdx.x;
    if (g >= W * Nout) return;
    uint32_t w = g / Nout, q = g % Nout;
    PT run = PT::inf(), t = PT::inf(), asum = PT::inf();
    for (int l = (int)m - 1; l >= 0; l--) {
        uint32_t j = q * m + (uint32_t)l;
        if (j >= N) continue;
        asum.add(PT::load(A_in + (size_t)w * N + j));
        run.add(PT::load(S_in + (size_t)w * N + j));
        if (l >= 1) t.add(run);
    }
    for (uint32_t i = 0; i < sh; i++) t.dbl();
    asum.add(t);
    asum.store(A_out + g);
    run.store(S_out + g);
}

template <class F, class PT = TailPt<F>>
__global__ __launch_bounds__(64) void k_reduce_wave(const XYZZ<F>* __restrict__ A_in, const XYZZ<F>* __restrict__ S_in, uint32_t N, uint32_t W,
                                                    uint32_t sh, XYZZ<F>* __restrict__ A_out, XYZZ<F>* __restrict__ S_out) {
    prio_hi();
    constexpr uint32_t FAN = 64 / PT::LPP;
    uint32_t Nout = (N + FAN - 1) / FAN;
    uint32_t chunk = blockIdx.x;
    uint32_t w = chunk / Nout, q = chunk % Nout;
    uint32_t lane = threadIdx.x / PT::LPP;
    uint32_t j = q * FAN + lane;
    PT s = PT::inf(), a = PT::inf();
    if (j < N) {
        s = PT::load(S_in + (size_t)w * N + j);
        a = PT::load(A_in + (size_t)w * N + j);
    }
    for (unsigned d = 1; d < FAN; d <<= 1) {
        PT t = s.shfl_down(d);
        if (lane + d < FAN) s.add(t);
    }
    PT y = s;
    if (lane == 0) y = PT::inf();
    for (uint32_t i = 0; i < sh; i++) y.dbl();
    y.add(a);
    for (unsigned d = FAN / 2; d > 0; d >>= 1) {
        PT t = y.shfl_xor(d);
        y.add(t);
    }
    if (threadIdx.x == 0) {
        s.store(S_out + chunk);
        y.store(A_out + chunk);
    }
}

#ifdef ZKMI_EXPERIMENTS
#include "experiments/msm_tail_fused.inc"
#endif

template <class HF> struct HostOf;
template <> struct HostOf<Fp> { typedef HFp type; };
template <> struct HostOf<Fp2> { typedef HFp2 type; };

unsigned msm_pick_window(size_t n) {
    unsigned best = 8;
    double bc = 1e300;
    for (unsigned c = 6; c <= 22; c++) {
        unsigned W = (255 + c - 1) / c;
        double cost = (double)n * W * 10.0 + (double)W * (double)((size_t)1 << (c - 1)) * 34.0;
        if (cost < bc) { bc = cost; best = c; }
    }
    return best;
}

unsigned msm_pick_window_table(size_t n) {
    unsigned best = 8;
    double bc = 1e300;
    const double lanes = 256.0 * 1024.0;
    for (unsigned c = 8; c <= 22; c++) {
        unsigned W = (255 + c - 1) / c;
        const double buckets = (double)((size_t)1 << (c - 1));
        const double eff = buckets >= lanes ? 1.0 : sqrt(sqrt(buckets / lanes));
        double cost = (double)n * W * 10.0 / eff + buckets * 34.0;
        if (cost < bc) { bc = cost; best = c; }
    }
    return best;
}

template <class F>
static int msm_plan_uncached(size_t n, const zk_msm_cfg* cfg, hipStream_t st, MsmPlan* P, const MsmTable* tab, unsigned sets);

template <class F>
static int msm_plan(size_t n, const zk_msm_cfg* cfg, hipStream_t st, MsmPlan* P, const MsmTable* tab = nullptr, unsigned sets = 1) {
    struct Key {
        size_t n, stride;
        unsigned c_cfg, c_tab, g2, l1, rows, sets;
        bool operator<(const Key& o) const { return std::tie(n, stride, c_cfg, c_tab, g2, l1, rows, sets) < std::tie(o.n, o.stride, o.c_cfg, o.c_tab, o.g2, o.l1, o.rows, o.sets); }
    };
    static std::mutex mu;
    static std::map<Key, MsmPlan> memo;
    Key k{n, tab ? tab->stride : 0, (cfg && cfg->window_bits) ? (unsigned)cfg->window_bits : 0u, tab ? tab->c : 0u, (unsigned)(sizeof(F) != 32), tab ? (tab->l1_m | (tab->l2_m << 8)) : 0u, tab ? (tab->row_first | (tab->row_step << 8)) : 0u, sets};
    {
        std::lock_guard<std::mutex> lk(mu);
        auto it = memo.find(k);
        if (it != memo.end()) { *P = it->second; return ZK_OK; }
    }
    ZK_TRY(msm_plan_uncached<F>(n, cfg, st, P, tab, sets));
    std::lock_guard<std::mutex> lk(mu);
    memo[k] = *P;
    return ZK_OK;
}

template <class F>
static int msm_plan_uncached(size_t n, const zk_msm_cfg* cfg, hipStream_t st, MsmPlan* P, const MsmTable* tab, unsigned sets) {
    typedef XYZZ<F> Pt;
    memset(P, 0, sizeof *P);
    if (n == 0) return ZK_OK;
    if (sets < 1 || sets > MSM_MAX_SETS || (sets > 1 && !tab)) return set_err(ZK_ERR_ARG, "a batch of %u scalar vectors needs a window table and at most %u vectors", sets, MSM_MAX_SETS);
    if (n > ((size_t)1 << 27)) return set_err(ZK_ERR_ARG, "n = %zu exceeds the per-call limit 2^27 (shard the MSM)", n);
    unsigned c = tab ? tab->c : ((cfg && cfg->window_bits) ? (unsigned)cfg->window_bits : msm_pick_window(n));
    if (c < 2 || c > (tab ? 24u : 22u)) return set_err(ZK_ERR_ARG, "window_bits = %u outside [2, %u]", c, tab ? 24u : 22u);
    P->c = c;
    P->Wd = (255 + c - 1) / c;
    P->W = tab ? sets : P->Wd;
    P->row_first = tab ? tab->row_first : 0;
    P->row_step = tab ? (tab->row_step ? tab->row_step : 1) : 1;
    P->Wrows = tab ? tab->rows() : P->Wd;
    if (tab && P->Wrows == 0) { memset(P, 0, sizeof *P); return ZK_OK; }
    P->table_stride = tab ? (uint32_t)tab->stride : 0;
    P->B = 1u << (c - 1);
    if ((uint64_t)P->W << (c - 1) >= ((uint64_t)1 << 30)) return set_err(ZK_ERR_ARG, "%u bucket sets of 2^%u buckets overflow the sort keys", P->W, c - 1);
    P->nb = P->W * P->B;
    P->total = n * P->Wrows * (tab ? sets : 1);
    if (P->total >= ((size_t)1 << 31)) return set_err(ZK_ERR_ARG, "n * windows = %zu overflows 31-bit positions", P->total);
    if (tab && (size_t)tab->stride * P->Wrows >= ((size_t)1 << 31)) return set_err(ZK_ERR_ARG, "table too large for 31-bit indices");
    size_t mean = P->total / P->nb + 1;
    {
        const uint64_t r_top64 = 0x30644e72e131a029ULL;
        unsigned shift = c * (P->Wd - 1);
        uint64_t top_max = shift >= 192 ? (r_top64 >> (shift - 192)) : ~0ULL;
        if (top_max < P->B && top_max > 0) {
            size_t dense = n / (size_t)top_max + 1 + (tab ? mean : 0);
            static const size_t dense_max = (size_t)ZK_EXP("ZKMI_L_DENSE", 4);
            if (dense > mean && dense <= dense_max * mean + 8 && dense_max) mean = dense;
        }
    }
    P->L = (uint32_t)(mean * 2 < 32 ? 32 : mean * 2);
    if (P->L < (n >> 16)) P->L = (uint32_t)(n >> 16);
    static const bool adaptive = (ZK_EXP("ZKMI_ADAPTIVE_L", 1) != 0);
    static const uint32_t lmin_div = (uint32_t)std::max<long>(1, ZK_EXP("ZKMI_L_MIN_DIV", 8));
    P->Lmin = adaptive ? (P->L / lmin_div > 32 ? P->L / lmin_div : 32) : P->L;
    if (P->Lmin > P->L) P->Lmin = P->L;
    P->max_tasks = (size_t)P->nb + P->total / P->Lmin + 1;
    static const unsigned l1_env = (unsigned)ZK_EXP("ZKMI_L1_M", 0);
    unsigned l1_m = l1_env ? l1_env : (tab && tab->l1_m ? tab->l1_m : 8);
    while (l1_m & (l1_m - 1)) l1_m &= l1_m - 1;
    P->m1 = P->B >= l1_m ? l1_m : P->B;
    P->m2 = (tab && tab->l2_m) ? tab->l2_m : 0;
    P->N1 = P->B / P->m1;
    P->key_bits = 1;
    while (((uint64_t)1 << P->key_bits) <= P->nb) P->key_bits++;
    P->sort_tmp_bytes = rs_plan(P->total, P->key_bits).tmp_bytes;
    P->scan_tmp_bytes = xs_tmp_bytes((size_t)P->nb + 1);
#ifdef ZKMI_EXPERIMENTS
#include "experiments/msm_sort_select.inc"
#endif
    P->lvl_elems = (size_t)P->W * P->N1;
    P->tsort_tmp_bytes = TS_BINS * 4;
    P->need_prep = 5 * align_up(P->max_tasks * 4, 256) + align_up(P->tsort_tmp_bytes + 16, 256) + 4 * align_up(P->total * 4, 256) +
                   align_up(P->sort_tmp_bytes + 16, 256) + align_up(P->scan_tmp_bytes + 16, 256) + 3 * align_up(((size_t)P->nb + 2) * 4, 256) +
                   align_up((size_t)P->nb * 4, 256) + 256 + 32768;
    P->need_acc = align_up(P->max_tasks * sizeof(Pt), 256) + 4 * align_up((P->lvl_elems + 64) * sizeof(Pt), 256) + 32768;
    P->need = P->need_prep + P->need_acc;
    return ZK_OK;
}

static int msm_prepare(Slot* s, hipStream_t st, const MsmPlan& P, const Fr* d_scalars, size_t n, const zk_msm_cfg* cfg, MsmPrep* out, const DigitSrc* batch = nullptr,
                       bool drop_zero_digits = false, const DigitRows* rows = nullptr) {
    out->P = P;
    out->n = n;
    out->empty = (n == 0) || P.total == 0;
    out->ready = nullptr;
    if (out->empty) return ZK_OK;
    const unsigned c = P.c, W = P.W, key_bits = P.key_bits;
    const uint32_t nb = P.nb, L = P.L;
    size_t total = P.total;
    const size_t max_tasks = P.max_tasks;
    size_t sort_tmp_bytes = P.sort_tmp_bytes, scan_tmp_bytes = P.scan_tmp_bytes;
    uint32_t* keys0 = (uint32_t*)s->alloc(total * 4);
    uint32_t* keys1 = (uint32_t*)s->alloc(total * 4);
    uint32_t* vals0 = (uint32_t*)s->alloc(total * 4);
    uint32_t* vals1 = (uint32_t*)s->alloc(total * 4);
    void* sort_tmp = s->alloc(sort_tmp_bytes + 16);
    void* scan_tmp = s->alloc(scan_tmp_bytes + 16);
    uint32_t* start = (uint32_t*)s->alloc(((size_t)nb + 2) * 4);
    uint32_t* ntasks = (uint32_t*)s->alloc(((size_t)nb + 2) * 4);
    uint32_t* task_off = (uint32_t*)s->alloc(((size_t)nb + 2) * 4);
    uint32_t* multi_list = (uint32_t*)s->alloc((size_t)nb * 4);
    uint32_t* task_begin = (uint32_t*)s->alloc(max_tasks * 4);
    uint32_t* lkey0 = (uint32_t*)s->alloc(max_tasks * 4);
    uint32_t* lkey1 = (uint32_t*)s->alloc(max_tasks * 4);
    uint32_t* tid1 = (uint32_t*)s->alloc(max_tasks * 4);
    uint32_t* bins = (uint32_t*)s->alloc(256 + TS_BINS * 4);
    if (!keys0 || !keys1 || !vals0 || !vals1 || !sort_tmp || !scan_tmp || !start || !ntasks || !task_off || !multi_list || !task_begin ||
        !lkey0 || !lkey1 || !tid1 || !bins)
        return set_err(ZK_ERR_HIP, "MSM workspace was not reserved up front (%zu bytes needed)", P.need_prep);
    uint32_t* num_multi = bins;
    uint32_t* hist = bins + 64;

    ZK_HIP(hipMemsetAsync(bins, 0, 256 + TS_BINS * 4, st));
    const uint32_t* d_total = nullptr;
    {
        DigitSrc src = batch ? *batch : DigitSrc{{d_scalars, nullptr, nullptr}};
        const unsigned sets = P.table_stride ? P.W : 1;
        const int mont = (cfg && cfg->scalars_mont) ? 1 : 0;
        const dim3 grid((unsigned)((n + 255) / 256), sets);
        if (drop_zero_digits && 256u * P.Wd * 8u > 65536u) drop_zero_digits = false;
        if (drop_zero_digits) {
            uint32_t* cnt = (uint32_t*)s->alloc(256);
            if (!cnt) return set_err(ZK_ERR_HIP, "MSM workspace was not reserved up front (zero-digit compaction)");
            ZK_HIP(hipMemsetAsync(cnt, 0, 4, st));
            if (rows) ZK_LAUNCH(s, st, "msm_digits", (k_msm_digits_compact<DigitRows>), grid, dim3(256), 256u * P.Wd * 8u, *rows, (uint32_t)n, mont, c, P.Wd, P.row_first, P.row_step,
                                P.table_stride, cnt, keys0, vals0);
            else ZK_LAUNCH(s, st, "msm_digits", (k_msm_digits_compact<DigitSrc>), grid, dim3(256), 256u * P.Wd * 8u, src, (uint32_t)n, mont, c, P.Wd, P.row_first, P.row_step, P.table_stride, cnt,
                           keys0, vals0);
            d_total = cnt;
        } else if (rows) {
            ZK_LAUNCH(s, st, "msm_digits", (k_msm_digits<DigitRows>), grid, dim3(256), 0, *rows, (uint32_t)n, mont, c, P.Wd, keys0, vals0, P.table_stride, P.row_first, P.row_step,
                      P.Wrows);
        } else {
            ZK_LAUNCH(s, st, "msm_digits", (k_msm_digits<DigitSrc>), grid, dim3(256), 0, src, (uint32_t)n, mont, c, P.Wd, keys0, vals0, P.table_stride, P.row_first, P.row_step,
                      P.Wrows);
        }
    }
    PingPong kb(keys0, keys1), vb(vals0, vals1);
    bool own_sort = true, own_scan = true;
#ifdef ZKMI_EXPERIMENTS
#include "experiments/msm_sort_rocprim_call.inc"
#endif
    if (own_sort) ZK_TRY(rs_sort_pairs(s, st, sort_tmp, kb, vb, total, key_bits, d_total));
    const uint32_t* keys = kb.current();
    ZK_LAUNCH(s, st, "msm_bucket_bounds", k_bucket_bounds, dim3((nb + 1 + 255) / 256), dim3(256), 0, keys, (uint32_t)total, nb, start, d_total);
    static const bool merged = ZK_EXP("ZKMI_PREP_MERGE", 1) != 0;
    static const uint32_t l_factor = (uint32_t)ZK_EXP("ZKMI_L_FACTOR", 4);
    static const uint32_t l_cap = (uint32_t)ZK_EXP("ZKMI_L_GIANT_CAP", 16384);
    static const uint32_t l_flat = (uint32_t)ZK_EXP("ZKMI_L_FLAT_KEEPS", 1);
    const unsigned stats_grid = nb / 4096 ? (nb / 4096 > 512 ? 512 : nb / 4096) : 1;
    const unsigned scan_tiles = (unsigned)(((size_t)nb + 1 + XS_TILE - 1) / XS_TILE);
    if (merged && P.Lmin < L) {
        ZK_LAUNCH(s, st, "msm_bucket_stats", k_bucket_stats_pick, dim3(stats_grid), dim3(256), 0, (const uint32_t*)start, nb, L, P.Lmin, (uint32_t)(ctx().num_cus * 1024), l_factor,
                  l_cap, l_flat, bins);
    } else {
        if (P.Lmin < L) ZK_LAUNCH(s, st, "msm_bucket_stats", k_bucket_stats, dim3(stats_grid), dim3(256), 0, (const uint32_t*)start, nb, bins);
        ZK_LAUNCH(s, st, "msm_pick_len", k_pick_len, dim3(1), dim3(1), 0, (const uint32_t*)start, nb, L, P.Lmin, (uint32_t)(ctx().num_cus * 1024), l_factor, l_cap, l_flat, bins);
    }
    if (merged && own_scan) {
        uint32_t* sums = (uint32_t*)scan_tmp;
        ZK_LAUNCH(s, st, "msm_task_plan", k_task_plan_scan, dim3(scan_tiles), dim3(XS_THREADS), 0, (const uint32_t*)start, nb, bins, ntasks, multi_list, sums);
        ZK_LAUNCH(s, st, "msm_task_scan", k_xs_apply, dim3(scan_tiles), dim3(XS_THREADS), 0, (const uint32_t*)ntasks, nb + 1, (const uint32_t*)sums, task_off);
    } else {
    ZK_LAUNCH(s, st, "msm_task_plan", k_task_plan, dim3((nb + 1 + 255) / 256), dim3(256), 0, (const uint32_t*)start, nb, (const uint32_t*)bins, ntasks, multi_list, num_multi);
#ifdef ZKMI_EXPERIMENTS
#include "experiments/msm_scan_rocprim_call.inc"
#endif
    if (own_scan) ZK_TRY(xs_exclusive_scan(s, st, scan_tmp, ntasks, task_off, (size_t)nb + 1));
    }
    uint32_t bshift = 0;
    while ((L >> bshift) >= TS_BINS) bshift++;
    const uint32_t nbins = (L >> bshift) + 1;
    const unsigned tgrid = (unsigned)((max_tasks + 255) / 256);
    static const bool merged_fill = ZK_EXP("ZKMI_PREP_MERGE", 1) == 2;
    if (merged_fill) {
        ZK_LAUNCH(s, st, "msm_task_fill", k_task_fill_bins, dim3(tgrid), dim3(256), 0, (const uint32_t*)start, (const uint32_t*)task_off, nb, L, bins, (uint32_t)max_tasks, bshift,
                  nbins, task_begin, lkey0, hist);
    } else {
        ZK_LAUNCH(s, st, "msm_task_fill", k_task_fill, dim3(tgrid), dim3(256), 0, (const uint32_t*)start, (const uint32_t*)task_off, nb, L, (const uint32_t*)bins,
                  (uint32_t)max_tasks, bshift, nbins, task_begin, lkey0, hist);
        ZK_LAUNCH(s, st, "msm_task_bins", k_task_bins, dim3(1), dim3(256), 0, hist, nbins);
    }
    ZK_LAUNCH(s, st, "msm_task_scatter", k_task_scatter, dim3(tgrid), dim3(256), 0, (const uint32_t*)lkey0, (uint32_t)max_tasks, bshift, nbins, hist,
              lkey1, tid1);
    out->vals = vb.current();
    out->keys = keys;
    out->d_total = d_total;
    out->start = start;
    out->task_off = task_off;
    out->task_begin = task_begin;
    out->lkeys = lkey1;
    out->tids = tid1;
    out->multi_list = multi_list;
    out->num_multi = num_multi;
    ZK_HIP(hipEventCreateWithFlags(&out->ready, hipEventDisableTiming));
    ZK_HIP(hipEventRecord(out->ready, st));
    return ZK_OK;
}

static int trace_copy(hipStream_t st, std::vector<unsigned char>& dst, const void* src, size_t bytes) {
    ZK_HIP(hipStreamSynchronize(st));
    dst.resize(bytes);
    if (bytes) ZK_HIP(hipMemcpy(dst.data(), src, bytes, hipMemcpyDeviceToHost));
    return ZK_OK;
}
static int trace_level(MsmTrace* tr, hipStream_t st, unsigned kind, uint32_t n_in, uint32_t n_out, uint32_t sh_in, uint32_t sh_out, uint32_t m, const void* A,
                       const void* S, size_t bytes) {
    tr->levels.emplace_back();
    MsmTraceLevel& lv = tr->levels.back();
    lv.kind = kind; lv.n_in = n_in; lv.n_out = n_out; lv.sh_in = sh_in; lv.sh_out = sh_out; lv.m = m;
    ZK_TRY(trace_copy(st, lv.A, A, bytes));
    return trace_copy(st, lv.S, S, bytes);
}

template <class F>
static int msm_accumulate_batch(int nb, Slot* const* sl, const hipStream_t* sts, const MsmPrep& R, const void* const* d_pts, const uint32_t* skip_below,
                                MsmJob* const* jobs) {
    typedef XYZZ<F> Pt;
    const MsmPlan& P = R.P;
    for (int b = 0; b < nb; b++) {
        jobs[b]->s = sl[b];
        jobs[b]->st = sts[b];
        jobs[b]->c = P.c;
        jobs[b]->W = P.W;
        jobs[b]->empty = R.empty;
    }
    if (R.empty) return ZK_OK;
    const unsigned W = P.W;
    const uint32_t B = P.B, L = P.L, m1 = P.m1, N1 = P.N1;
    const size_t max_tasks = P.max_tasks, lvl_elems = P.lvl_elems;
    Pt *partial[3], *lvlA[3][2], *lvlS[3][2];
    AccBatch batch = {};
    for (int b = 0; b < nb; b++) {
        Slot* s = sl[b];
        partial[b] = (Pt*)s->alloc(max_tasks * sizeof(Pt));
        for (int k = 0; k < 2; k++) {
            lvlA[b][k] = (Pt*)s->alloc((lvl_elems + 64) * sizeof(Pt));
            lvlS[b][k] = (Pt*)s->alloc((lvl_elems + 64) * sizeof(Pt));
        }
        if (!partial[b] || !lvlA[b][0] || !lvlA[b][1] || !lvlS[b][0] || !lvlS[b][1])
            return set_err(ZK_ERR_HIP, "MSM workspace was not reserved up front (%zu bytes needed)", P.need_acc);
        batch.pts[b] = d_pts[b];
        batch.partial[b] = partial[b];
        batch.skip_below[b] = skip_below[b];
    }
    MsmJob* j0 = jobs[0];
    hipStream_t sa = j0->chain ? j0->chain : sts[0];
    if (R.ready) ZK_HIP(hipStreamWaitEvent(sa, R.ready, 0));
    if (j0->gate_acc) ZK_HIP(hipStreamWaitEvent(sa, j0->gate_acc, 0));
    struct Turnstile {
        std::mutex mu;
        hipEvent_t ring[16] = {};
        int next = 0;
        hipEvent_t last = nullptr;
    };
    static Turnstile g_turn[MAX_ENTRIES];
    Turnstile* T = j0->turnstile ? &g_turn[current_entry()] : nullptr;
    std::unique_lock<std::mutex> turn_lock;
    if (T) {
        turn_lock = std::unique_lock<std::mutex>(T->mu);
        if (T->last) ZK_HIP(hipStreamWaitEvent(sa, T->last, 0));
    }
    const char* acc_name = sizeof(F) == 32 ? "msm_accumulate_g1" : "msm_accumulate_g2";
    const unsigned full_grid = (unsigned)((max_tasks + 255) / 256);
    bool launched = false;
    const bool tab = P.table_stride != 0;
    for (int b = 0; tab && b < nb; b++)
        if (skip_below[b]) return set_err(ZK_ERR_ARG, "skip_below is for the plain method (a table's entries are not point indices)");
#ifdef ZKMI_EXPERIMENTS
    if (!tab) {
#include "experiments/msm_accumulate_variants_launch.inc"
    }
#endif
    static const unsigned acc_lds_kb = (unsigned)ZK_EXP("ZKMI_ACC_LDS_KB", 0);
    static const unsigned acc_lds_min_tasks = (unsigned)ZK_EXP("ZKMI_ACC_LDS_MIN_TASKS", 0);
    unsigned acc_shmem = (acc_lds_kb && max_tasks >= acc_lds_min_tasks) ? acc_lds_kb * 1024u : 0u;
    if (acc_shmem > 65536u) {
        static std::mutex attr_mu;
        static uint64_t attr_done = 0;
        std::lock_guard<std::mutex> lk(attr_mu);
        if (!(attr_done & ((uint64_t)1 << current_entry()))) {
            ZK_HIP(hipFuncSetAttribute(reinterpret_cast<const void*>(k_accumulate<Fp>), hipFuncAttributeMaxDynamicSharedMemorySize, 160 * 1024));
            ZK_HIP(hipFuncSetAttribute(reinterpret_cast<const void*>(k_accumulate<Fp2>), hipFuncAttributeMaxDynamicSharedMemorySize, 160 * 1024));
            ZK_HIP(hipFuncSetAttribute(reinterpret_cast<const void*>(k_accumulate<Fp, true>), hipFuncAttributeMaxDynamicSharedMemorySize, 160 * 1024));
            ZK_HIP(hipFuncSetAttribute(reinterpret_cast<const void*>(k_accumulate<Fp2, true>), hipFuncAttributeMaxDynamicSharedMemorySize, 160 * 1024));
            attr_done |= (uint64_t)1 << current_entry();
        }
    }
// ... 109 lines not shown
    if (per_set)
        for (unsigned w = 0; w < (job.empty ? 3u : job.W); w++) per_set[w] = XYZZ<HF>::inf();
    if (job.empty) return ZK_OK;
    ZK_TRY(slot_sync(job.s, job.st));
    const unsigned N = job.n_final;
    if constexpr (sizeof(HF) == sizeof(HFp)) {
        static const HFp inv32 = HFp{{32, 0, 0, 0}}.to_mont().inv();
        XYZZ<HFp>* w = reinterpret_cast<XYZZ<HFp>*>(job.s->pinned);
        const size_t cnt = (size_t)job.W * N * (N > 1 ? 2 : 1);
        for (size_t i = 0; i < cnt; i++) {
            w[i].x = w[i].x * inv32;
            w[i].y = w[i].y * inv32;
            w[i].zz = w[i].zz * inv32;
            w[i].zzz = w[i].zzz * inv32;
        }
    }
    const XYZZ<HF>* wa = reinterpret_cast<const XYZZ<HF>*>(job.s->pinned);
    const XYZZ<HF>* wsum = wa + (size_t)job.W * N;
    XYZZ<HF> tot = XYZZ<HF>::inf();
    for (int w = (int)job.W - 1; w >= 0; w--) {
        for (unsigned k = 0; k < job.c; k++) tot.dbl();
        XYZZ<HF> val = wa[(size_t)w * N];
        if (N > 1) {
            XYZZ<HF> run = XYZZ<HF>::inf(), acc = XYZZ<HF>::inf();
            for (unsigned j = N - 1; j >= 1; j--) {
                run.add(wsum[(size_t)w * N + j]);
                acc.add(run);
                val.add(wa[(size_t)w * N + j]);
            }
            for (unsigned k = 0; k < job.sh_final; k++) acc.dbl();
            val.add(acc);
        }
        if (per_set) per_set[w] = val;
        tot.add(val);
    }
    *total_out = tot;
    return ZK_OK;
}

__device__ __forceinline__ Fp fp_inv_chain(const Fp& z) {
    Fp acc = Fp::one(), base = z;
#pragma unroll
    for (int w = 0; w < 8; w++) {
        uint32_t e = FpParams::MOD[w] - (w == 0 ? 2u : 0u);
#pragma unroll 1
        for (int b = 0; b < 32; b++) {
            if (e & 1u) acc = acc * base;
            base = base.sqr();
            e >>= 1;
        }
    }
    return acc;
}
__global__ __launch_bounds__(64) void k_msm_sets_affine(const XYZZ<Fp>* __restrict__ A_in, const XYZZ<Fp>* __restrict__ S_in, uint32_t N, uint32_t sh, uint32_t sets,
                                                       Affine<Fp>* __restrict__ out, uint32_t* __restrict__ compressed) {
    prio_hi();
    const uint32_t w = blockIdx.x * blockDim.x + threadIdx.x;
    if (w >= sets) return;
    Affine<Fp> a = Affine<Fp>::inf();
    if (N) {
        typedef TailPt<Fp> PT;
        const XYZZ<Fp>* A = A_in + (size_t)w * N;
        PT val = PT::load(A);
        if (N > 1) {
            const XYZZ<Fp>* S = S_in + (size_t)w * N;
            PT run = PT::inf(), acc = PT::inf();
#pragma unroll 1
            for (uint32_t j = N - 1; j >= 1; j--) {
                run.add(PT::load(S + j));
                acc.add(run);
                val.add(PT::load(A + j));
            }
#pragma unroll 1
            for (uint32_t k = 0; k < sh; k++) acc.dbl();
            val.add(acc);
        }
        const XYZZ<Fp> r = acc29_to_xyzz(val.v);
        if (!r.is_inf()) {
            const Fp t = fp_inv_chain(r.zz * r.zzz);
            a.x = r.x * (t * r.zzz);
            a.y = r.y * (t * r.zz);
        }
    }
    if (out) gstore(out + w, a);
    if (compressed) {
        uint32_t raw[8];
        g1_compress_one(a, raw);
#pragma unroll
        for (int k = 0; k < 8; k++) compressed[(size_t)w * 8 + k] = raw[k];
    }
}
int msm_g1_sets_affine_dev(const MsmJob& job, unsigned sets, void* d_out, void* d_compressed) {
    if (!sets || (!d_out && !d_compressed)) return ZK_OK;
    if (!job.s || !job.st) return set_err(ZK_ERR_ARG, "the job was not launched");
    if (((uintptr_t)d_compressed & 3) || ((uintptr_t)d_out & 15)) return set_err(ZK_ERR_ARG, "d_out must be 16-byte and d_compressed 4-byte aligned");
    if (!job.empty) {
        if (!job.keep_final || !job.d_final_a || !job.d_final_s) return set_err(ZK_ERR_ARG, "the job did not keep its last level on the device");
        if (job.W != sets) return set_err(ZK_ERR_ARG, "the job holds %u bucket sets, not %u", job.W, sets);
    }
    ZK_LAUNCH(job.s, job.st, "msm_sets_affine", k_msm_sets_affine, dim3((sets + 63) / 64), dim3(64), 0, (const XYZZ<Fp>*)job.d_final_a, (const XYZZ<Fp>*)job.d_final_s,
              job.empty ? 0u : job.n_final, job.sh_final, (uint32_t)sets, (Affine<Fp>*)d_out, (uint32_t*)d_compressed);
    return ZK_OK;
}

int msm_g1_need(size_t n, const zk_msm_cfg* cfg, hipStream_t st, size_t* need) {
    MsmPlan P;
    ZK_TRY(msm_plan<Fp>(n, cfg, st, &P));
    *need = P.need;
    return ZK_OK;
}
int msm_g2_need(size_t n, const zk_msm_cfg* cfg, hipStream_t st, size_t* need) {
    MsmPlan P;
    ZK_TRY(msm_plan<Fp2>(n, cfg, st, &P));
    *need = P.need;
    return ZK_OK;
}
int msm_g1_launch(Slot* s, hipStream_t st, const void* d_pts, const void* d_scalars, size_t n, const zk_msm_cfg* cfg, MsmJob* job) {
    MsmPlan P;
    ZK_TRY(msm_plan<Fp>(n, cfg, st, &P));
    return msm_launch<Fp>(s, st, P, (const Affine<Fp>*)d_pts, (const Fr*)d_scalars, n, cfg, job);
}
int msm_g2_launch(Slot* s, hipStream_t st, const void* d_pts, const void* d_scalars, size_t n, const zk_msm_cfg* cfg, MsmJob* job) {
    MsmPlan P;
    ZK_TRY(msm_plan<Fp2>(n, cfg, st, &P));
    return msm_launch<Fp2>(s, st, P, (const Affine<Fp2>*)d_pts, (const Fr*)d_scalars, n, cfg, job);
}
int msm_prep_need(size_t n, const zk_msm_cfg* cfg, hipStream_t st, size_t* need_prep, size_t* need_acc_g1, size_t* need_acc_g2) {
    MsmPlan P1, P2;
    ZK_TRY(msm_plan<Fp>(n, cfg, st, &P1));
    ZK_TRY(msm_plan<Fp2>(n, cfg, st, &P2));
    if (need_prep) *need_prep = P1.need_prep;
    if (need_acc_g1) *need_acc_g1 = P1.need_acc;
    if (need_acc_g2) *need_acc_g2 = P2.need_acc;
    return ZK_OK;
}
int msm_prep_need_table(size_t n, const MsmTable& tab, hipStream_t st, size_t* need_prep, size_t* need_acc_g1, size_t* need_acc_g2) {
    MsmPlan P1, P2;
    ZK_TRY(msm_plan<Fp>(n, nullptr, st, &P1, &tab));
    ZK_TRY(msm_plan<Fp2>(n, nullptr, st, &P2, &tab));
    if (need_prep) *need_prep = P1.need_prep;
    if (need_acc_g1) *need_acc_g1 = P1.need_acc;
    if (need_acc_g2) *need_acc_g2 = P2.need_acc;
    return ZK_OK;
}
int msm_prep_need_table_batch(size_t n, unsigned sets, const MsmTable& tab, hipStream_t st, size_t* need_prep, size_t* need_acc_g1) {
    MsmPlan P1;
    ZK_TRY(msm_plan<Fp>(n, nullptr, st, &P1, &tab, sets));
    if (need_prep) *need_prep = P1.need_prep;
    if (need_acc_g1) *need_acc_g1 = P1.need_acc;
    return ZK_OK;
}
size_t msm_compact_need(size_t, unsigned) { return 1024; }
int msm_prepare_scalars_table_batch(Slot* s, hipStream_t st, const void* const* d_scalars, unsigned sets, size_t n, const zk_msm_cfg* cfg, const MsmTable& tab, MsmPrep* out,
                                    bool drop_zero_digits) {
    if (sets < 1 || sets > 3) return set_err(ZK_ERR_ARG, "a batch holds one to three scalar vectors");
    MsmPlan P;
    ZK_TRY(msm_plan<Fp>(n, cfg, st, &P, &tab, sets));
    DigitSrc src = {{nullptr, nullptr, nullptr}};
    for (unsigned v = 0; v < sets; v++) src.p[v] = (const Fr*)d_scalars[v];
    return msm_prepare(s, st, P, src.p[0], n, cfg, out, &src, drop_zero_digits);
}
int msm_prep_need_table_rows(size_t n, unsigned sets, const MsmTable& tab, hipStream_t st, size_t* need_prep, size_t* need_acc_g1, size_t* need_acc_g2) {
    MsmPlan P1, P2;
    ZK_TRY(msm_plan<Fp>(n, nullptr, st, &P1, &tab, sets));
    ZK_TRY(msm_plan<Fp2>(n, nullptr, st, &P2, &tab, sets));
    if (need_prep) *need_prep = P1.need_prep;
    if (need_acc_g1) *need_acc_g1 = P1.need_acc;
    if (need_acc_g2) *need_acc_g2 = P2.need_acc;
    return ZK_OK;
}
int msm_prepare_scalars_table_rows(Slot* s, hipStream_t st, const void* d_base, size_t row_stride, unsigned sets, size_t n, const zk_msm_cfg* cfg, const MsmTable& tab,
                                   MsmPrep* out, bool drop_zero_digits) {
    MsmPlan P;
    ZK_TRY(msm_plan<Fp>(n, cfg, st, &P, &tab, sets));
    const DigitRows rows = {(const Fr*)d_base, row_stride};
    return msm_prepare(s, st, P, rows.base, n, cfg, out, nullptr, drop_zero_digits, &rows);
}
int msm_prepare_scalars_table(Slot* s, hipStream_t st, const void* d_scalars, size_t n, const zk_msm_cfg* cfg, const MsmTable& tab, MsmPrep* out, bool drop_zero_digits) {
    MsmPlan P;
    ZK_TRY(msm_plan<Fp>(n, cfg, st, &P, &tab));
    return msm_prepare(s, st, P, (const Fr*)d_scalars, n, cfg, out, nullptr, drop_zero_digits);
}

template <class F>
__global__ __launch_bounds__(256) void k_build_table(const Affine<F>* __restrict__ pts, uint32_t n, uint32_t stride, uint32_t offset, unsigned c,
                                                     unsigned Wd, unsigned row_first, unsigned row_step, TabPt<F>* __restrict__ table) {
    uint32_t i = blockIdx.x * blockDim.x + threadIdx.x;
    if (i >= n) return;
    Affine<F> p = gload(pts + i);
    if (p.is_inf()) return;
    constexpr int MAXR = 32;
    F xs[MAXR], ys[MAXR], zs[MAXR], ws[MAXR], pre[MAXR];
    int k = 0;
    if constexpr (std::is_same<F, Fp>::value) {
        {
            Acc29 A;
            acc29_from_xyzz(A, XYZZ<Fp>::from_affine(p));
            for (unsigned w = 0; w < Wd; w++) {
                if (w) {
                    for (unsigned b = 0; b < c; b++) acc29_dbl(A);
                }
                if (w < row_first || (w - row_first) % row_step) continue;
                const XYZZ<Fp> r = acc29_to_xyzz(A);
                xs[k] = r.x; ys[k] = r.y; zs[k] = r.zz; ws[k] = r.zzz;
                k++;
            }
        }
    }
    if constexpr (std::is_same<F, Fp2>::value) {
        Acc29G2 A;
        acc29g2_from_xyzz(A, XYZZ<Fp2>::from_affine(p));
        for (unsigned w = 0; w < Wd; w++) {
            if (w) {
                for (unsigned b = 0; b < c; b++) acc29g2_dbl(A);
            }
            if (w < row_first || (w - row_first) % row_step) continue;
            const XYZZ<Fp2> r = acc29g2_to_xyzz(A);
            xs[k] = r.x; ys[k] = r.y; zs[k] = r.zz; ws[k] = r.zzz;
            k++;
        }
    }
    if (k == 0) {
        XYZZ<F> acc = XYZZ<F>::from_affine(p);
        for (unsigned w = 0; w < Wd; w++) {
            if (w) {
                for (unsigned b = 0; b < c; b++) acc.dbl();
            }
            if (w < row_first || (w - row_first) % row_step) continue;
            xs[k] = acc.x; ys[k] = acc.y; zs[k] = acc.zz; ws[k] = acc.zzz;
            k++;
        }
    }
    F run = F::one();
    for (int j = 0; j < k; j++) {
        pre[j] = run;
        run = run * (zs[j] * ws[j]);
    }
    if (run.is_zero()) {
        for (int j = 0; j < k; j++) {
            const Affine<F> a = XYZZ<F>{xs[j], ys[j], zs[j], ws[j]}.to_affine();
            if (!a.is_inf()) gstore(table + (size_t)j * stride + offset + i, tab29_make(a));
        }
        return;
    }
    F inv = run.inv();
    for (int j = k - 1; j >= 0; j--) {
        const F t = inv * pre[j];
        inv = inv * (zs[j] * ws[j]);
        Affine<F> a{xs[j] * (t * ws[j]), ys[j] * (t * zs[j])};
        gstore(table + (size_t)j * stride + offset + i, tab29_make(a));
    }
}
size_t msm_table_entry_bytes(int is_g2) { return is_g2 ? sizeof(TabPt<Fp2>) : sizeof(TabPt<Fp>); }
template <class F>
static int build_table(Slot* s, hipStream_t st, const void* d_pts, size_t n, size_t stride, size_t offset, unsigned c, void* d_table, unsigned row_first,
                       unsigned row_step) {
    MsmTable t;
    t.c = c; t.row_first = row_first; t.row_step = row_step ? row_step : 1;
    unsigned Wd = (255 + c - 1) / c, rows = t.rows();
    ZK_HIP(hipMemsetAsync(d_table, 0, (size_t)(rows ? rows : 1) * stride * sizeof(TabPt<F>), st));
    if (n && rows)
        ZK_LAUNCH(s, st, sizeof(F) == 32 ? "msm_build_table_g1" : "msm_build_table_g2", (k_build_table<F>), dim3((unsigned)((n + 255) / 256)), dim3(256), 0,
                  (const Affine<F>*)d_pts, (uint32_t)n, (uint32_t)stride, (uint32_t)offset, c, Wd, row_first, t.row_step, (TabPt<F>*)d_table);
    return ZK_OK;
}
int msm_build_table_g1(Slot* s, hipStream_t st, const void* d_pts, size_t n, size_t stride, size_t offset, unsigned c, void* d_table, unsigned row_first,
                       unsigned row_step) {
    return build_table<Fp>(s, st, d_pts, n, stride, offset, c, d_table, row_first, row_step);
}
int msm_build_table_g2(Slot* s, hipStream_t st, const void* d_pts, size_t n, size_t stride, size_t offset, unsigned c, void* d_table, unsigned row_first,
                       unsigned row_step) {
    return build_table<Fp2>(s, st, d_pts, n, stride, offset, c, d_table, row_first, row_step);
}

template <class F>
__global__ __launch_bounds__(256) void k_expand_bases(const Affine<F>* __restrict__ compact, const uint32_t* __restrict__ src_idx, uint32_t n,
                                                      Affine<F>* __restrict__ out) {
    uint32_t i = blockIdx.x * blockDim.x + threadIdx.x;
    if (i >= n) return;
    uint32_t j = src_idx[i];
    Affine<F> p;
    uint4* d = reinterpret_cast<uint4*>(&p);
    if (j == 0xffffffffu) {
#pragma unroll
        for (unsigned k = 0; k < sizeof(p) / 16; k++) d[k] = make_uint4(0, 0, 0, 0);
    } else {
        p = gload(compact + j);
    }
    gstore(out + i, p);
}
int msm_expand_bases(Slot* s, hipStream_t st, int is_g2, const void* d_compact, const uint32_t* d_src_idx, size_t n, void* d_out) {
    if (!n) return ZK_OK;
    if (is_g2)
        ZK_LAUNCH(s, st, "pk_expand_bases_g2", (k_expand_bases<Fp2>), dim3((unsigned)((n + 255) / 256)), dim3(256), 0, (const Affine<Fp2>*)d_compact, d_src_idx,
                  (uint32_t)n, (Affine<Fp2>*)d_out);
    else
        ZK_LAUNCH(s, st, "pk_expand_bases_g1", (k_expand_bases<Fp>), dim3((unsigned)((n + 255) / 256)), dim3(256), 0, (const Affine<Fp>*)d_compact, d_src_idx,
                  (uint32_t)n, (Affine<Fp>*)d_out);
    return ZK_OK;
}

int msm_prepare_scalars(Slot* s, hipStream_t st, const void* d_scalars, size_t n, const zk_msm_cfg* cfg, MsmPrep* out, bool drop_zero_digits) {
    MsmPlan P;
    ZK_TRY(msm_plan<Fp>(n, cfg, st, &P));
    return msm_prepare(s, st, P, (const Fr*)d_scalars, n, cfg, out, nullptr, drop_zero_digits);
}
void msm_prep_release(MsmPrep* R) {
    if (R->ready) (void)hipEventDestroy(R->ready);
    R->ready = nullptr;
}
int msm_g1_accumulate(Slot* s, hipStream_t st, const MsmPrep& R, const void* d_pts, uint32_t skip_below, MsmJob* job) {
    return msm_accumulate<Fp>(s, st, R, (const Affine<Fp>*)d_pts, skip_below, job);
}
int msm_g1_accumulate_batch(int nb, Slot* const* sl, const hipStream_t* sts, const MsmPrep& R, const void* const* d_pts, const uint32_t* skip_below,
                            MsmJob* const* jobs) {
    if (nb < 1 || nb > 3) return set_err(ZK_ERR_ARG, "accumulate batch of %d", nb);
    return msm_accumulate_batch<Fp>(nb, sl, sts, R, d_pts, skip_below, jobs);
}
int msm_g2_accumulate(Slot* s, hipStream_t st, const MsmPrep& R, const void* d_pts, uint32_t skip_below, MsmJob* job) {
    return msm_accumulate<Fp2>(s, st, R, (const Affine<Fp2>*)d_pts, skip_below, job);
}
int msm_g1_finish(const MsmJob& job, XYZZ<HFp>* out) { return msm_finish<HFp>(job, out); }
int msm_g1_finish_batch(const MsmJob& job, XYZZ<HFp> out[3]) {
    XYZZ<HFp> unused;
    return msm_finish<HFp>(job, &unused, out);
}
int msm_g2_finish(const MsmJob& job, XYZZ<HFp2>* out) { return msm_finish<HFp2>(job, out); }
int msm_g1_finish_sets(const MsmJob& job, XYZZ<HFp>* out, unsigned sets) {
    XYZZ<HFp> unused;
    for (unsigned k = 0; k < sets; k++) out[k] = XYZZ<HFp>::inf();
    if (!job.empty && job.W != sets) return set_err(ZK_ERR_ARG, "the job holds %u bucket sets, not %u", job.W, sets);
    return msm_finish<HFp>(job, &unused, out);
}
// ... 15 lines not shown
}

static int check_cfg(const zk_msm_cfg* cfg) {
    if (cfg && cfg->nb_tasks > 1024) return set_err(ZK_ERR_NB_TASKS, "invalid config: config.NbTasks > 1024");
    return ZK_OK;
}

struct Bases {
    void* d = nullptr;
    size_t n = 0;
    int is_g2 = 0;
    void* d_table = nullptr;
    MsmTable tab;
};
static std::mutex g_bases_mu;
static std::map<uint64_t, Bases> g_bases;
static uint64_t g_next_handle = 1;

int bases_ptr(uint64_t handle, const void** d, size_t* n, int* is_g2) {
    std::lock_guard<std::mutex> lk(g_bases_mu);
    auto it = g_bases.find(handle);
    if (it == g_bases.end()) return set_err(ZK_ERR_HANDLE, "unknown bases handle %llu", (unsigned long long)handle);
    if (d) *d = it->second.d;
    if (n) *n = it->second.n;
    if (is_g2) *is_g2 = it->second.is_g2;
    return ZK_OK;
}
int bases_table(uint64_t handle, const void** d_table, MsmTable* tab, size_t* n) {
    if (md_is_composite(handle)) {
        if (d_table) *d_table = nullptr;
        return md_bases_info(handle, n, nullptr);
    }
    std::lock_guard<std::mutex> lk(g_bases_mu);
    auto it = g_bases.find(handle);
    if (it == g_bases.end()) return set_err(ZK_ERR_HANDLE, "unknown bases handle %llu", (unsigned long long)handle);
    if (d_table) *d_table = it->second.d_table;
    if (tab) *tab = it->second.tab;
    if (n) *n = it->second.n;
    return ZK_OK;
}
int bases_info(uint64_t handle, size_t* n, int* is_g2) {
    if (md_is_composite(handle)) return md_bases_info(handle, n, is_g2);
    std::lock_guard<std::mutex> lk(g_bases_mu);
    auto it = g_bases.find(handle);
    if (it == g_bases.end()) return set_err(ZK_ERR_HANDLE, "unknown bases handle %llu", (unsigned long long)handle);
    if (n) *n = it->second.n;
    if (is_g2) *is_g2 = it->second.is_g2;
    return ZK_OK;
}

}

using namespace zkmi;

template <class HF, class OUT>
static void write_affine(const XYZZ<HF>& t, OUT* out) {
    Affine<HF> a = t.to_affine();
    memcpy(out, &a, sizeof(a));
}

template <int G2>
static int msm_host_impl(const void* points, size_t n_points, const zk_fr* scalars, size_t n_scalars, const zk_msm_cfg* cfg, void* out) {
    const size_t psz = G2 ? 128 : 64;
    if (n_points != n_scalars) return set_err(ZK_ERR_LEN, "len(points) != len(scalars)");
    ZK_TRY(check_cfg(cfg));
    if (!out || (n_points && (!points || !scalars))) return set_err(ZK_ERR_ARG, "null pointer");
    SlotGuard g;
    ZK_TRY(acquire_slot(&g.s));
    hipStream_t st = g.s->stream;
    size_t n = n_points, need = 0;
    ZK_TRY(G2 ? msm_g2_need(n, cfg, st, &need) : msm_g1_need(n, cfg, st, &need));
    ZK_TRY(g.s->reserve(n * (psz + 32) + 1024 + need));
    void* d_p = g.s->alloc(n * psz + 16);
    void* d_s = g.s->alloc(n * 32 + 16);
    if (n) {
        ZK_HIP(hipMemcpyAsync(d_p, points, n * psz, hipMemcpyHostToDevice, st));
        ZK_HIP(hipMemcpyAsync(d_s, scalars, n * 32, hipMemcpyHostToDevice, st));
    }
    if (G2) {
        XYZZ<HFp2> t;
        ZK_TRY(msm_g2_xyzz(g.s, st, d_p, d_s, n, cfg, &t));
        write_affine(t, (zk_g2_affine*)out);
    } else {
        XYZZ<HFp> t;
        ZK_TRY(msm_g1_xyzz(g.s, st, d_p, d_s, n, cfg, &t));
        write_affine(t, (zk_g1_affine*)out);
    }
    return ZK_OK;
}

template <int G2>
static int msm_dev_impl(const void* d_points, const void* d_scalars, size_t n, const zk_msm_cfg* cfg, void* out, void* stream, int partial) {
    ZK_TRY(check_cfg(cfg));
    if (!out || (n && (!d_points || !d_scalars))) return set_err(ZK_ERR_ARG, "null pointer");
    SlotGuard g;
    ZK_TRY(acquire_slot(&g.s));
    hipStream_t st = stream ? (hipStream_t)stream : g.s->stream;
    size_t need = 0;
    ZK_TRY(G2 ? msm_g2_need(n, cfg, st, &need) : msm_g1_need(n, cfg, st, &need));
    ZK_TRY(g.s->reserve(need));
    if (G2) {
        XYZZ<HFp2> t;
        ZK_TRY(msm_g2_xyzz(g.s, st, d_points, d_scalars, n, cfg, &t));
        if (partial) memcpy(out, &t, sizeof(t)); else write_affine(t, (zk_g2_affine*)out);
    } else {
        XYZZ<HFp> t;
        ZK_TRY(msm_g1_xyzz(g.s, st, d_points, d_scalars, n, cfg, &t));
        if (partial) memcpy(out, &t, sizeof(t)); else write_affine(t, (zk_g1_affine*)out);
    }
    return ZK_OK;
}

template <int G2>
static int msm_host_entry(const void* points, size_t n_points, const zk_fr* scalars, size_t n_scalars, const zk_msm_cfg* cfg, void* out) {
    if (n_points != n_scalars) return set_err(ZK_ERR_LEN, "len(points) != len(scalars)");
    ZK_TRY(check_cfg(cfg));
    if (!out || (n_points && (!points || !scalars))) return set_err(ZK_ERR_ARG, "null pointer");
    std::vector<int> ents;
    ZK_TRY(md_entries_for(cfg ? (uint32_t)cfg->device_mask : 0u, n_points, (size_t)1 << 17, &ents));
    if (ents.size() > 1 && n_points >= ents.size()) return md_msm_host(G2, points, scalars, n_points, cfg, out, ents);
    CtxScope sc(ents[0]);
    if (sc.rc != ZK_OK) return sc.rc;
    return msm_host_impl<G2>(points, n_points, scalars, n_scalars, cfg, out);
}
extern "C" {

int zk_bn254_msm_plan_info(size_t n, int window_tables, uint32_t* window_bits, uint32_t* digits) {
    if (!window_bits || !digits) return set_err(ZK_ERR_ARG, "null pointer");
    unsigned c = window_tables ? msm_pick_window_table(n) : msm_pick_window(n);
    *window_bits = c;
    *digits = (255 + c - 1) / c;
    return ZK_OK;
}

static int msm_prep_inspect_run(Slot* s, const zk_msm_prep_request* q, const zk_msm_cfg* cfg, const MsmTable* tab, const MsmPlan& P, MsmPrep* prep,
                                zk_msm_prep_result* r, size_t extra = 0, bool allow_empty = false) {
    hipStream_t st = s->stream;
    const size_t n = q->n;
    const unsigned sets = tab ? q->sets : 1;
    const size_t elems = q->by_rows ? (size_t)(sets - 1) * q->row_stride + n : n;
    ZK_TRY(s->reserve((q->by_rows ? 1 : sets) * (elems * 32 + 256) + P.need_prep + msm_compact_need(n, sets) + 4096 + extra));
    const void* d_vec[3] = {nullptr, nullptr, nullptr};
    for (unsigned v = 0; v < (q->by_rows ? 1u : sets) && P.total; v++) {
        for (unsigned u = 0; u < v; u++)
            if (q->vec[u] == q->vec[v]) d_vec[v] = d_vec[u];
        if (d_vec[v]) continue;
        void* d = s->alloc(elems * 32 + 16);
        if (!d) return set_err(ZK_ERR_HIP, "MSM inspection: scalar buffer was not reserved");
        ZK_HIP(hipMemcpyAsync(d, q->vec[v], elems * 32, hipMemcpyHostToDevice, st));
        d_vec[v] = d;
    }
    const bool drop = q->drop_zero_digits != 0;
    if (!tab) ZK_TRY(msm_prepare_scalars(s, st, d_vec[0], n, cfg, prep, drop));
    else if (q->by_rows) ZK_TRY(msm_prepare_scalars_table_rows(s, st, d_vec[0], q->row_stride, sets, n, cfg, *tab, prep, drop));
    else if (sets > 1) ZK_TRY(msm_prepare_scalars_table_batch(s, st, d_vec, sets, n, cfg, *tab, prep, drop));
    else ZK_TRY(msm_prepare_scalars_table(s, st, d_vec[0], n, cfg, *tab, prep, drop));
    if (prep->empty && allow_empty && P.total == 0) return ZK_OK;
    if (prep->empty) return set_err(ZK_ERR_ARG, "MSM inspection: the preparation is empty where its plan is not");
    ZK_HIP(hipStreamSynchronize(st));
    auto back = [&](uint32_t* dst, const uint32_t* src, size_t count) -> int {
        if (dst && count) ZK_HIP(hipMemcpy(dst, src, count * 4, hipMemcpyDeviceToHost));
        return ZK_OK;
    };
    uint32_t dev_total = (uint32_t)P.total;
    if (prep->d_total) ZK_HIP(hipMemcpy(&dev_total, prep->d_total, 4, hipMemcpyDeviceToHost));
    r->device_total = dev_total;
    r->dropped = prep->d_total ? 1u : 0u;
    ZK_HIP(hipMemcpy(r->ctl, prep->num_multi, sizeof r->ctl, hipMemcpyDeviceToHost));
    ZK_TRY(back(r->keys, prep->keys, P.total));
    ZK_TRY(back(r->vals, prep->vals, P.total));
    ZK_TRY(back(r->start, prep->start, (size_t)P.nb + 1));
    ZK_TRY(back(r->task_off, prep->task_off, (size_t)P.nb + 1));
    ZK_TRY(back(r->task_begin, prep->task_begin, P.max_tasks));
    ZK_TRY(back(r->len_keys, prep->lkeys, P.max_tasks));
    ZK_TRY(back(r->task_ids, prep->tids, P.max_tasks));
    ZK_TRY(back(r->multi_list, prep->multi_list, P.nb));
    return ZK_OK;
}
static int msm_inspect_plan(const zk_msm_prep_request* q, unsigned l1_m, unsigned l2_m, zk_msm_cfg* cfg, MsmTable* tab, MsmPlan* P, zk_msm_prep_result* r) {
    memset(cfg, 0, sizeof *cfg);
    cfg->scalars_mont = q->scalars_mont;
    cfg->window_bits = q->window_bits;
    if (q->table) {
        if (q->sets < 1 || (!q->by_rows && q->sets > 3)) return set_err(ZK_ERR_ARG, "MSM inspection: one to three vectors by pointer, any number by rows");
        if (q->stride < q->n || (q->by_rows && q->sets > 1 && q->row_stride < q->n)) return set_err(ZK_ERR_ARG, "MSM inspection: a stride shorter than the vectors");
        tab->c = q->c;
        tab->stride = q->stride;
        tab->row_first = q->row_first;
        tab->row_step = q->row_step ? q->row_step : 1;
        tab->l1_m = l1_m;
        tab->l2_m = l2_m;
    } else if (q->sets > 1 || q->by_rows) {
        return set_err(ZK_ERR_ARG, "MSM inspection: several vectors need table mode");
    }
    ZK_TRY(msm_plan<Fp>(q->n, cfg, nullptr, P, q->table ? tab : nullptr, q->table ? q->sets : 1));
    r->c = P->c; r->W = P->W; r->Wd = P->Wd; r->Wrows = P->Wrows; r->B = P->B; r->nb = P->nb; r->key_bits = P->key_bits; r->L = P->L; r->Lmin = P->Lmin;
    r->m1 = P->m1; r->N1 = P->N1; r->dropped = 0;
    r->total = P->total; r->max_tasks = P->max_tasks; r->device_total = 0;
    memset(r->ctl, 0, sizeof r->ctl);
    return ZK_OK;
}
static bool msm_prep_sizes_only(const zk_msm_prep_result* r) {
    return !r->keys && !r->vals && !r->start && !r->task_off && !r->task_begin && !r->len_keys && !r->task_ids && !r->multi_list;
}
int zk_bn254_msm_prep_inspect(const zk_msm_prep_request* q, zk_msm_prep_result* r) {
    if (!q || !r) return set_err(ZK_ERR_ARG, "null pointer");
    zk_msm_cfg cfg;
    MsmTable tab;
    MsmPlan P;
    ZK_TRY(msm_inspect_plan(q, 0, 0, &cfg, &tab, &P, r));
    if (msm_prep_sizes_only(r) || P.total == 0) return ZK_OK;
    for (unsigned v = 0; v < (q->by_rows ? 1u : (q->table ? q->sets : 1u)); v++)
        if (!q->vec[v]) return set_err(ZK_ERR_ARG, "null pointer");
    SlotGuard g;
    ZK_TRY(acquire_slot(&g.s));
    MsmPrep prep;
    int rc = msm_prep_inspect_run(g.s, q, &cfg, q->table ? &tab : nullptr, P, &prep, r);
    if (rc != ZK_OK) (void)hipStreamSynchronize(g.s->stream);
    msm_prep_release(&prep);
    return rc;
}

static unsigned msm_tail_geometry(const MsmPlan& P, bool quad, zk_msm_tail_level* lv, uint32_t* n_final, uint32_t* sh_final) {
    unsigned k = 0;
    uint32_t N = P.N1, sh = 0;
    for (uint32_t mm = P.m1; mm > 1; mm >>= 1) sh++;
    lv[k++] = zk_msm_tail_level{MsmTraceLevel::L1, P.B, P.N1, 0, sh, P.m1};
    if (P.m2 > 1 && N > 64 * P.m2) {
        uint32_t Nout = (N + P.m2 - 1) / P.m2, sh_in = sh;
        for (uint32_t mm = P.m2; mm > 1; mm >>= 1) sh++;
        lv[k++] = zk_msm_tail_level{MsmTraceLevel::L2, N, Nout, sh_in, sh, P.m2};
        N = Nout;
    }
    const uint32_t fan = quad ? 16 : 64, fan_log = quad ? 4 : 6, host_n = P.W == 1 ? 64 : 1;
    while (N > host_n && k < ZK_MSM_TAIL_MAX_LEVELS) {
        uint32_t Nout = (N + fan - 1) / fan;
        lv[k++] = zk_msm_tail_level{quad ? (uint32_t)MsmTraceLevel::WAVE_QUAD : (uint32_t)MsmTraceLevel::WAVE, N, Nout, sh, sh + fan_log, fan};
        N = Nout;
        sh += fan_log;
    }
    *n_final = N;
    *sh_final = sh;
    return k;
}
}
template <class HF>
static void tail_affine(const unsigned char* raw, size_t count, uint64_t* out) {
    static const HFp inv32 = HFp{{32, 0, 0, 0}}.to_mont().inv();
    for (size_t i = 0; i < count; i++) {
        XYZZ<HF> p;
        memcpy(&p, raw + i * sizeof p, sizeof p);
        if constexpr (sizeof(HF) == sizeof(HFp)) {
            p.x = p.x * inv32;
            p.y = p.y * inv32;
            p.zz = p.zz * inv32;
            p.zzz = p.zzz * inv32;
        }
        Affine<HF> a = p.to_affine();
        memcpy(out + i * (sizeof a / 8), &a, sizeof a);
    }
}
static void table_affine(const uint64_t* rows, size_t count, unsigned nc, uint64_t* out) {
    static const HFp inv32 = HFp{{32, 0, 0, 0}}.to_mont().inv();
    for (size_t i = 0; i < count; i++) {
        const uint64_t* e = rows + i * nc * 4;
        uint64_t* o = out + i * nc * 4;
        if (!(e[(nc / 2) * 4 + 3] >> 63)) {
            memset(o, 0, nc * 32);
            continue;
        }
        for (unsigned k = 0; k < nc; k++) {
            HFp v;
            memcpy(&v, e + k * 4, 32);
            v.l[3] &= ~((uint64_t)1 << 63);
            v = v * inv32;
            memcpy(o + k * 4, &v, 32);
        }
    }
}
struct DevFree {
    void* p = nullptr;
    ~DevFree() { if (p) (void)hipFree(p); }
};
template <int G2>
static int msm_tail_inspect_run(Slot* s, const zk_msm_tail_request* q, const zk_msm_cfg* cfg, const MsmTable* tab, const MsmPlan& P, size_t need_acc, MsmPrep* prep,
                                zk_msm_tail_result* r) {
    typedef typename std::conditional<G2 != 0, HFp2, HFp>::type HF;
    const size_t psz = G2 ? 128 : 64, aw = psz / 8, n = q->prep.n;
    const unsigned sets = tab ? q->prep.sets : 1;
    hipStream_t st = s->stream;
    DevFree d_pts, d_tab;
    ZK_HIP(hipMalloc(&d_pts.p, n * psz + 256));
    if (n) ZK_HIP(hipMemcpyAsync(d_pts.p, q->points, n * psz, hipMemcpyHostToDevice, st));
    const size_t tab_entries = (size_t)r->table_entries;
    if (tab) {
        const size_t tsz = msm_table_entry_bytes(G2);
        const size_t tab_alloc = ((size_t)std::max(tab->rows(), 1u) * tab->stride + 1) * tsz;
        ZK_HIP(hipMalloc(&d_tab.p, tab_alloc));
        ZK_HIP(hipMemsetAsync(d_tab.p, 0, tab_alloc, st));
        ZK_TRY(G2 ? msm_build_table_g2(s, st, d_pts.p, n, tab->stride, 0, tab->c, d_tab.p, tab->row_first, tab->row_step)
                  : msm_build_table_g1(s, st, d_pts.p, n, tab->stride, 0, tab->c, d_tab.p, tab->row_first, tab->row_step));
        if (r->table && tab_entries) {
            ZK_HIP(hipStreamSynchronize(st));
            std::vector<uint64_t> rows(tab_entries * (tsz / 8));
            ZK_HIP(hipMemcpy(rows.data(), d_tab.p, tab_entries * tsz, hipMemcpyDeviceToHost));
            table_affine(rows.data(), tab_entries, G2 ? 4 : 2, r->table);
        }
    }
    ZK_TRY(msm_prep_inspect_run(s, &q->prep, cfg, tab, P, prep, &r->prep, need_acc + (size_t)sets * 128 + 4096, true));
    uint32_t tasks = 0;
    if (!prep->empty) ZK_HIP(hipMemcpy(&tasks, prep->task_off + P.nb, 4, hipMemcpyDeviceToHost));
    MsmTrace trace;
    MsmJob job;
    job.trace = &trace;
    job.quad_tail = q->quad_tail != 0;
    job.keep_final = q->keep_final != 0;
    const void* d_bases = tab ? d_tab.p : d_pts.p;
    ZK_TRY(G2 ? msm_g2_accumulate(s, st, *prep, d_bases, q->skip_below, &job) : msm_g1_accumulate(s, st, *prep, d_bases, q->skip_below, &job));
    if (q->keep_final) {
        if constexpr (!G2) {
            void* d_out = s->alloc((size_t)sets * 64);
            void* d_enc = s->alloc((size_t)sets * 32);
            if (!d_out || !d_enc) return set_err(ZK_ERR_HIP, "MSM inspection: the finisher's buffers were not reserved");
            ZK_TRY(msm_g1_sets_affine_dev(job, sets, d_out, d_enc));
            ZK_TRY(slot_sync(s, st));
            if (r->final_affine) ZK_HIP(hipMemcpy(r->final_affine, d_out, (size_t)sets * 64, hipMemcpyDeviceToHost));
            if (r->final_bytes) ZK_HIP(hipMemcpy(r->final_bytes, d_enc, (size_t)sets * 32, hipMemcpyDeviceToHost));
        }
    } else {
        std::vector<XYZZ<HF>> per_set(std::max(P.W, 3u));
        XYZZ<HF> tot = XYZZ<HF>::inf();
        if (!tab) {
            ZK_TRY(msm_finish<HF>(job, &tot, per_set.data()));
        } else {
            if constexpr (G2) ZK_TRY(msm_g2_finish_sets(job, per_set.data(), sets));
            else ZK_TRY(msm_g1_finish_sets(job, per_set.data(), sets));
        }
        if (r->total && !tab) write_affine(tot, r->total);
        for (unsigned w = 0; r->set_values && w < P.W; w++) write_affine(per_set[w], r->set_values + (size_t)w * aw);
    }
    if (job.empty) return ZK_OK;
    bool same = job.n_final == r->n_final && job.sh_final == r->sh_final && trace.levels.size() == r->n_levels;
    for (unsigned k = 0; same && k < r->n_levels; k++) {
        const MsmTraceLevel& a = trace.levels[k];
        const zk_msm_tail_level& b = r->level[k];
        same = a.kind == b.kind && a.n_in == b.n_in && a.n_out == b.n_out && a.sh_in == b.sh_in && a.sh_out == b.sh_out && a.m == b.m;
    }
    if (!same) return set_err(ZK_ERR_ARG, "MSM inspection: the tail ran %zu levels to n_final = %u, sh_final = %u; the plan states %u, %u, %u", trace.levels.size(),
                              job.n_final, job.sh_final, r->n_levels, r->n_final, r->sh_final);
    r->tasks = tasks;
    if (r->partial_acc) tail_affine<HF>(trace.partial_acc.data(), tasks, r->partial_acc);
    if (r->partial_fold) tail_affine<HF>(trace.partial_fold.data(), tasks, r->partial_fold);
    size_t at = 0;
    for (const MsmTraceLevel& lv : trace.levels) {
        const size_t cnt = (size_t)P.W * lv.n_out;
        if (r->level_a) tail_affine<HF>(lv.A.data(), cnt, r->level_a + at * aw);
        if (r->level_s) tail_affine<HF>(lv.S.data(), cnt, r->level_s + at * aw);
        at += cnt;
    }
    return ZK_OK;
}
extern "C" {
int zk_bn254_msm_tail_inspect(const zk_msm_tail_request* q, zk_msm_tail_result* r) {
    if (!q || !r) return set_err(ZK_ERR_ARG, "null pointer");
    const zk_msm_prep_request* pq = &q->prep;
    if (q->is_g2 && (q->quad_tail || q->keep_final)) return set_err(ZK_ERR_ARG, "MSM inspection: the four-lane tail and the device finish are G1 only");
    if (!pq->table && (q->l1_m || q->l2_m || q->keep_final)) return set_err(ZK_ERR_ARG, "MSM inspection: level sizes and the device finish need table mode");
    if (pq->table && q->skip_below) return set_err(ZK_ERR_ARG, "MSM inspection: skip_below is for the plain method (a table's entries are not point indices)");
    zk_msm_cfg cfg;
    MsmTable tab;
    MsmPlan P;
    ZK_TRY(msm_inspect_plan(pq, q->l1_m, q->l2_m, &cfg, &tab, &P, &r->prep));
    size_t need_acc = P.need_acc;
    if (q->is_g2) {
        MsmPlan P2;
        ZK_TRY(msm_plan<Fp2>(pq->n, &cfg, nullptr, &P2, pq->table ? &tab : nullptr, pq->table ? pq->sets : 1));
        need_acc = P2.need_acc;
    }
    r->m2 = P.m2;
    r->tasks = 0;
    r->table_entries = pq->table ? (uint64_t)tab.rows() * tab.stride : 0;
    memset(r->level, 0, sizeof r->level);
    r->n_levels = P.total ? msm_tail_geometry(P, q->quad_tail != 0, r->level, &r->n_final, &r->sh_final) : 0;
    if (!P.total) r->n_final = r->sh_final = 0;
    r->level_entries = 0;
    for (unsigned k = 0; k < r->n_levels; k++) r->level_entries += (uint64_t)P.W * r->level[k].n_out;
    const bool sizes_only = msm_prep_sizes_only(&r->prep) && !r->table && !r->partial_acc && !r->partial_fold && !r->level_a && !r->level_s && !r->set_values &&
                            !r->total && !r->final_affine && !r->final_bytes;
    if (sizes_only) return ZK_OK;
    if (P.total == 0 && !q->keep_final) return ZK_OK;
    if (pq->n && !q->points) return set_err(ZK_ERR_ARG, "null pointer");
    for (unsigned v = 0; P.total && v < (pq->by_rows ? 1u : (pq->table ? pq->sets : 1u)); v++)
        if (!pq->vec[v]) return set_err(ZK_ERR_ARG, "null pointer");
    SlotGuard g;
    ZK_TRY(acquire_slot(&g.s));
    MsmPrep prep;
    int rc = q->is_g2 ? msm_tail_inspect_run<1>(g.s, q, &cfg, pq->table ? &tab : nullptr, P, need_acc, &prep, r)
                      : msm_tail_inspect_run<0>(g.s, q, &cfg, pq->table ? &tab : nullptr, P, need_acc, &prep, r);
    if (rc != ZK_OK) (void)hipStreamSynchronize(g.s->stream);
    msm_prep_release(&prep);
    return rc;
}

int zk_bn254_g1_msm(const zk_g1_affine* points, size_t n_points, const zk_fr* scalars, size_t n_scalars, const zk_msm_cfg* cfg, zk_g1_affine* out) {
    return msm_host_entry<0>(points, n_points, scalars, n_scalars, cfg, out);
}
int zk_bn254_g2_msm(const zk_g2_affine* points, size_t n_points, const zk_fr* scalars, size_t n_scalars, const zk_msm_cfg* cfg, zk_g2_affine* out) {
    return msm_host_entry<1>(points, n_points, scalars, n_scalars, cfg, out);
}
int zk_bn254_g1_msm_dev(const void* d_points, const void* d_scalars, size_t n, const zk_msm_cfg* cfg, zk_g1_affine* out_host, void* stream) {
    return msm_dev_impl<0>(d_points, d_scalars, n, cfg, out_host, stream, 0);
}
int zk_bn254_g2_msm_dev(const void* d_points, const void* d_scalars, size_t n, const zk_msm_cfg* cfg, zk_g2_affine* out_host, void* stream) {
    return msm_dev_impl<1>(d_points, d_scalars, n, cfg, out_host, stream, 0);
}
int zk_bn254_g1_msm_partial_dev(const void* d_points, const void* d_scalars, size_t n, const zk_msm_cfg* cfg, uint64_t out_xyzz[16], void* stream) {
    return msm_dev_impl<0>(d_points, d_scalars, n, cfg, out_xyzz, stream, 1);
}
int zk_bn254_g2_msm_partial_dev(const void* d_points, const void* d_scalars, size_t n, const zk_msm_cfg* cfg, uint64_t out_xyzz[32], void* stream) {
    return msm_dev_impl<1>(d_points, d_scalars, n, cfg, out_xyzz, stream, 1);
}
int zk_bn254_g1_sum_xyzz(const uint64_t* partials, size_t n_partials, zk_g1_affine* out) {
    if (!out || (n_partials && !partials)) return set_err(ZK_ERR_ARG, "null pointer");
    XYZZ<HFp> t = XYZZ<HFp>::inf();
    for (size_t i = 0; i < n_partials; i++) {
        XYZZ<HFp> p;
        memcpy(&p, partials + 16 * i, sizeof(p));
        t.add(p);
    }
    write_affine(t, out);
    return ZK_OK;
}
int zk_bn254_g2_sum_xyzz(const uint64_t* partials, size_t n_partials, zk_g2_affine* out) {
    if (!out || (n_partials && !partials)) return set_err(ZK_ERR_ARG, "null pointer");
    XYZZ<HFp2> t = XYZZ<HFp2>::inf();
    for (size_t i = 0; i < n_partials; i++) {
        XYZZ<HFp2> p;
        memcpy(&p, partials + 32 * i, sizeof(p));
        t.add(p);
    }
    write_affine(t, out);
    return ZK_OK;
}

static int bases_register_here(const void* points, size_t n, int is_g2, uint64_t* handle, hipMemcpyKind kind, int table_c);
static int bases_register(const void* points, size_t n, int is_g2, uint64_t* handle, hipMemcpyKind kind, int table_c) {
    if (!handle || (n && !points)) return set_err(ZK_ERR_ARG, "null pointer");
    if (table_c != 0 && table_c != -1 && (table_c < 8 || table_c > 24)) return set_err(ZK_ERR_ARG, "table_window_bits = %d outside [8, 24]", table_c);
    ZK_TRY(ensure_init());
    if (md_default_mask()) {
        std::vector<int> ents;
        ZK_TRY(md_entries_for(0, n, (size_t)1 << 16, &ents));
        if (ents.size() > 1) return md_bases_register(points, n, is_g2, kind == hipMemcpyDeviceToDevice, table_c, ents, handle);
    }
    return bases_register_here(points, n, is_g2, handle, kind, table_c);
}
}
namespace zkmi {
int bases_register_on_this_entry(const void* points, size_t n, int is_g2, int on_device, int table_c, uint64_t* handle) {
    return bases_register_here(points, n, is_g2, handle, on_device ? hipMemcpyDeviceToDevice : hipMemcpyHostToDevice, table_c);
}
}
static int bases_make_table(Bases* b, int table_c) {
    const size_t n = b->n;
    const int is_g2 = b->is_g2;
    MsmTable tab;
    tab.c = table_c > 0 ? (unsigned)table_c : msm_pick_window_table(n);
    tab.stride = n;
    tab.l1_m = (unsigned)ZK_EXP("ZKMI_BASES_L1M", 0);
    tab.l2_m = (unsigned)ZK_EXP("ZKMI_BASES_L2M", 0);
    const size_t Wd = (255 + tab.c - 1) / tab.c, tbytes = Wd * n * msm_table_entry_bytes(is_g2);
    size_t free_b = 0, total_b = 0;
    ZK_HIP(hipMemGetInfo(&free_b, &total_b));
    if (tbytes < free_b / 2 && tbytes <= ((size_t)64 << 30)) {
        SlotGuard g;
        ZK_TRY(acquire_slot(&g.s));
        void* d_table = nullptr;
        ZK_HIP(hipMalloc(&d_table, tbytes));
        int rc = is_g2 ? msm_build_table_g2(g.s, g.s->stream, b->d, n, n, 0, tab.c, d_table) : msm_build_table_g1(g.s, g.s->stream, b->d, n, n, 0, tab.c, d_table);
        if (rc == ZK_OK) rc = slot_sync(g.s, g.s->stream);
        if (rc != ZK_OK) { (void)hipFree(d_table); return rc; }
        b->tab = tab;
        b->d_table = d_table;
    } else if (table_c > 0) {
        return set_err(ZK_ERR_HIP, "window tables of %zu bytes do not fit (free HBM %zu)", tbytes, free_b);
    }
    return ZK_OK;
}
extern "C" {
static int bases_register_here(const void* points, size_t n, int is_g2, uint64_t* handle, hipMemcpyKind kind, int table_c) {
    if (!handle || (n && !points)) return set_err(ZK_ERR_ARG, "null pointer");
    if (table_c != 0 && table_c != -1 && (table_c < 8 || table_c > 24)) return set_err(ZK_ERR_ARG, "table_window_bits = %d outside [8, 24]", table_c);
    ZK_TRY(ensure_init());
    Bases b;
    b.n = n;
    b.is_g2 = is_g2 ? 1 : 0;
    size_t bytes = n * (is_g2 ? 128 : 64);
    ZK_HIP(hipMalloc(&b.d, bytes ? bytes : 16));
    struct Cleanup {
        Bases* b;
        ~Cleanup() { if (b) { (void)hipFree(b->d); if (b->d_table) (void)hipFree(b->d_table); } }
    } cleanup{&b};
    if (bytes) ZK_HIP(hipMemcpy(b.d, points, bytes, kind));
    if (n && table_c != -1 && (table_c > 0 || n >= 4096)) ZK_TRY(bases_make_table(&b, table_c));
    std::lock_guard<std::mutex> lk(g_bases_mu);
    *handle = hmake(g_next_handle++);
    g_bases[*handle] = b;
    cleanup.b = nullptr;
    return ZK_OK;
}
int zk_bn254_bases_register(const void* points, size_t n, int is_g2, uint64_t* handle) { return bases_register(points, n, is_g2, handle, hipMemcpyHostToDevice, 0); }
int zk_bn254_bases_register_dev(const void* d_points, size_t n, int is_g2, uint64_t* handle) {
    return bases_register(d_points, n, is_g2, handle, hipMemcpyDeviceToDevice, 0);
}
int zk_bn254_bases_register_cfg(const void* points, size_t n, int is_g2, int on_device, int table_window_bits, uint64_t* handle) {
    return bases_register(points, n, is_g2, handle, on_device ? hipMemcpyDeviceToDevice : hipMemcpyHostToDevice, table_window_bits);
}
int zk_bn254_bases_free(uint64_t handle) {
    if (md_is_composite(handle)) return md_bases_free(handle);
    ZK_ON_ENTRY_OF(handle);
    std::lock_guard<std::mutex> lk(g_bases_mu);
    auto it = g_bases.find(handle);
    if (it == g_bases.end()) return set_err(ZK_ERR_HANDLE, "unknown bases handle %llu", (unsigned long long)handle);
    (void)hipFree(it->second.d);
    if (it->second.d_table) (void)hipFree(it->second.d_table);
    g_bases.erase(it);
    return ZK_OK;
}
int zk_bn254_bases_build_table(uint64_t handle, int table_window_bits) {
// ... 476 lines not shown
```

noir_backend_using_gnark_amd/csrc/msm.hpp:

```cpp
#pragma once
#include "ctx.hpp"
#include "curve.hpp"
#include "host_ff.hpp"
#include <vector>

namespace zkmi {

unsigned msm_pick_window(size_t n);
int msm_g1_need(size_t n, const zk_msm_cfg* cfg, hipStream_t st, size_t* need);
int msm_g2_need(size_t n, const zk_msm_cfg* cfg, hipStream_t st, size_t* need);
struct MsmTable {
    unsigned c = 0;
    size_t stride = 0;
    unsigned row_first = 0, row_step = 1;
    unsigned rows() const {
        unsigned Wd = (255 + c - 1) / c;
        return row_first < Wd ? (Wd - 1 - row_first) / row_step + 1 : 0;
    }
    unsigned l2_m = 0;
    unsigned l1_m = 0;
};
unsigned msm_pick_window_table(size_t n);
size_t msm_table_entry_bytes(int is_g2);
int msm_build_table_g1(Slot* s, hipStream_t st, const void* d_pts, size_t n, size_t stride, size_t offset, unsigned c, void* d_table, unsigned row_first = 0,
                       unsigned row_step = 1);
int msm_build_table_g2(Slot* s, hipStream_t st, const void* d_pts, size_t n, size_t stride, size_t offset, unsigned c, void* d_table, unsigned row_first = 0,
                       unsigned row_step = 1);

int msm_expand_bases(Slot* s, hipStream_t st, int is_g2, const void* d_compact, const uint32_t* d_src_idx, size_t n, void* d_out);

int bases_info(uint64_t handle, size_t* n, int* is_g2);
struct MsmTable;
int bases_table(uint64_t handle, const void** d_table, MsmTable* tab, size_t* n);

struct MsmPlan {
    unsigned c, W, Wd, key_bits;
    unsigned Wrows, row_first, row_step;
    uint32_t table_stride;
    uint32_t B, nb, L, m1, N1, m2 = 0;
    uint32_t Lmin = 0;
    size_t total, max_tasks, sort_tmp_bytes, scan_tmp_bytes, tsort_tmp_bytes, lvl_elems, need, need_prep, need_acc;
};
struct MsmPrep {
    MsmPlan P;
    size_t n = 0;
    bool empty = true;
    const uint32_t *vals = nullptr, *start = nullptr, *task_off = nullptr, *task_begin = nullptr, *lkeys = nullptr, *tids = nullptr,
                   *multi_list = nullptr, *num_multi = nullptr;
    const uint32_t *keys = nullptr;
    const uint32_t *d_total = nullptr;
    hipEvent_t ready = nullptr;
};

struct MsmTraceLevel {
    enum Kind : unsigned { L1 = 1, L2 = 2, WAVE = 3, WAVE_QUAD = 4 };
    unsigned kind = 0;
    uint32_t n_in = 0, n_out = 0;
    uint32_t sh_in = 0, sh_out = 0;
    uint32_t m = 0;
    std::vector<unsigned char> A, S;
};
struct MsmTrace {
    std::vector<unsigned char> partial_acc, partial_fold;
    std::vector<MsmTraceLevel> levels;
};

struct MsmJob {
    Slot* s = nullptr;
    hipStream_t st = nullptr;
    unsigned c = 0, W = 0;
    unsigned n_final = 1, sh_final = 0;
    bool empty = true;
    hipEvent_t gate_acc = nullptr;
    bool want_done = false;
    hipEvent_t acc_done = nullptr;
    hipStream_t chain = nullptr;
    bool turnstile = false;
    bool quad_tail = false;
    bool keep_final = false;
    const void *d_final_a = nullptr, *d_final_s = nullptr;
    MsmTrace* trace = nullptr;
};
int msm_g1_sets_affine_dev(const MsmJob& job, unsigned sets, void* d_out, void* d_compressed);
int msm_g1_launch(Slot* s, hipStream_t st, const void* d_pts, const void* d_scalars, size_t n, const zk_msm_cfg* cfg, MsmJob* job);
int msm_g2_launch(Slot* s, hipStream_t st, const void* d_pts, const void* d_scalars, size_t n, const zk_msm_cfg* cfg, MsmJob* job);
int msm_prep_need(size_t n, const zk_msm_cfg* cfg, hipStream_t st, size_t* need_prep, size_t* need_acc_g1, size_t* need_acc_g2);
int msm_prepare_scalars(Slot* s, hipStream_t st, const void* d_scalars, size_t n, const zk_msm_cfg* cfg, MsmPrep* out, bool drop_zero_digits = false);
int msm_prep_need_table(size_t n, const MsmTable& tab, hipStream_t st, size_t* need_prep, size_t* need_acc_g1, size_t* need_acc_g2);
int msm_prepare_scalars_table(Slot* s, hipStream_t st, const void* d_scalars, size_t n, const zk_msm_cfg* cfg, const MsmTable& tab, MsmPrep* out, bool drop_zero_digits = false);
int msm_prep_need_table_batch(size_t n, unsigned sets, const MsmTable& tab, hipStream_t st, size_t* need_prep, size_t* need_acc_g1);
int msm_prepare_scalars_table_batch(Slot* s, hipStream_t st, const void* const* d_scalars, unsigned sets, size_t n, const zk_msm_cfg* cfg, const MsmTable& tab, MsmPrep* out,
                                    bool drop_zero_digits = false);
static constexpr unsigned MSM_MAX_SETS = 1024;
int msm_prep_need_table_rows(size_t n, unsigned sets, const MsmTable& tab, hipStream_t st, size_t* need_prep, size_t* need_acc_g1, size_t* need_acc_g2);
int msm_prepare_scalars_table_rows(Slot* s, hipStream_t st, const void* d_base, size_t row_stride, unsigned sets, size_t n, const zk_msm_cfg* cfg, const MsmTable& tab,
                                   MsmPrep* out, bool drop_zero_digits = false);
int msm_g1_finish_sets(const MsmJob& job, XYZZ<HFp>* out, unsigned sets);
int msm_g2_finish_sets(const MsmJob& job, XYZZ<HFp2>* out, unsigned sets);
size_t msm_compact_need(size_t n, unsigned sets);
int msm_bases_batch_dev_sparse(uint64_t handle, size_t offset, const void* const* d_scalars, unsigned count, size_t n, const zk_msm_cfg* cfg, void* out);
int msm_g1_finish_batch(const MsmJob& job, XYZZ<HFp> out[3]);
void msm_prep_release(MsmPrep* R);
int msm_g1_accumulate(Slot* s, hipStream_t st, const MsmPrep& R, const void* d_pts, uint32_t skip_below, MsmJob* job);
int msm_g2_accumulate(Slot* s, hipStream_t st, const MsmPrep& R, const void* d_pts, uint32_t skip_below, MsmJob* job);
int msm_g1_accumulate_batch(int nb, Slot* const* sl, const hipStream_t* sts, const MsmPrep& R, const void* const* d_pts, const uint32_t* skip_below,
                            MsmJob* const* jobs);
int msm_g1_finish(const MsmJob& job, XYZZ<HFp>* out);
int msm_g2_finish(const MsmJob& job, XYZZ<HFp2>* out);
int msm_g1_xyzz(Slot* s, hipStream_t st, const void* d_pts, const void* d_scalars, size_t n, const zk_msm_cfg* cfg, XYZZ<HFp>* out);
int msm_g2_xyzz(Slot* s, hipStream_t st, const void* d_pts, const void* d_scalars, size_t n, const zk_msm_cfg* cfg, XYZZ<HFp2>* out);

}
```

Measured before the change: 450.9 million G1 scalar-muls/s (whole prove: 4 G1 MSMs + G2 MSM + 7 NTTs per step).

## Spread top-window digits by adding multiples of the modulus to scalars

In table mode, scalars whose top window is nonzero get k·r added, with k = i mod K, using a 9-limb representation. This spreads the top-window digits evenly across buckets instead of crowding the low buckets that the modulus limit allows. The plan drops the special top-window bucket-skew handling when spread is on, and spread defaults to true for table-based preparation. The cost is slightly more digit-extraction arithmetic, and correctness depends on the point order equalling r so that k·r contributes nothing.

```diff
diff --git a/include/zkmi.h b/include/zkmi.h
--- a/include/zkmi.h
+++ b/include/zkmi.h
@@ -331,7 +331,7 @@
     int window_bits, scalars_mont, table, drop_zero_digits;
     uint32_t c, row_first, row_step, sets;
     size_t stride;
-    int by_rows, reserved;
+    int by_rows, spread;
     const zk_fr *vec[3];
     size_t row_stride;
 } zk_msm_prep_request;
@@ -340,6 +340,7 @@
     uint64_t total, max_tasks, device_total;
     uint32_t ctl[64];
     uint32_t *keys, *vals, *start, *task_off, *task_begin, *len_keys, *task_ids, *multi_list;
+    uint32_t spread_K, reserved;
 } zk_msm_prep_result;
 int zk_bn254_msm_prep_inspect(const zk_msm_prep_request *req, zk_msm_prep_result *res);
 
diff --git a/noir_backend_using_gnark_amd/_lib.py b/noir_backend_using_gnark_amd/_lib.py
--- a/noir_backend_using_gnark_amd/_lib.py
+++ b/noir_backend_using_gnark_amd/_lib.py
@@ -30,7 +30,7 @@
 class MsmPrepRequest(C.Structure):
     _fields_ = [("n", C.c_size_t), ("window_bits", C.c_int), ("scalars_mont", C.c_int), ("table", C.c_int), ("drop_zero_digits", C.c_int),
                 ("c", C.c_uint32), ("row_first", C.c_uint32), ("row_step", C.c_uint32), ("sets", C.c_uint32), ("stride", C.c_size_t),
-                ("by_rows", C.c_int), ("reserved", C.c_int), ("vec", C.c_void_p * 3), ("row_stride", C.c_size_t)]
+                ("by_rows", C.c_int), ("spread", C.c_int), ("vec", C.c_void_p * 3), ("row_stride", C.c_size_t)]
 
 
 MSM_PREP_PLAN = ("c", "W", "Wd", "Wrows", "B", "nb", "key_bits", "L", "Lmin", "m1", "N1")
@@ -39,7 +39,8 @@
 
 class MsmPrepResult(C.Structure):
     _fields_ = [(k, C.c_uint32) for k in MSM_PREP_PLAN + ("dropped",)] + [("total", C.c_uint64), ("max_tasks", C.c_uint64), ("device_total", C.c_uint64),
-                                                                         ("ctl", C.c_uint32 * 64)] + [(k, C.c_void_p) for k in MSM_PREP_ARRAYS]
+                                                                         ("ctl", C.c_uint32 * 64)] + [(k, C.c_void_p) for k in MSM_PREP_ARRAYS] + \
+               [("spread_K", C.c_uint32), ("reserved", C.c_uint32)]
 
 
 MSM_TAIL_MAX_LEVELS = 12
diff --git a/noir_backend_using_gnark_amd/bn254.py b/noir_backend_using_gnark_amd/bn254.py
--- a/noir_backend_using_gnark_amd/bn254.py
+++ b/noir_backend_using_gnark_amd/bn254.py
@@ -81,7 +81,7 @@
     return out
 
 
-def _msm_prep_request(req, vectors, n, window_bits, scalars_mont, table_c, stride, row_first, row_step, rows, row_stride, drop_zero_digits):
+def _msm_prep_request(req, vectors, n, window_bits, scalars_mont, table_c, stride, row_first, row_step, rows, row_stride, drop_zero_digits, spread=False):
     if rows:
         mat = _as_u64(vectors, 4)
         row_stride = row_stride if row_stride is not None else mat.shape[0] // rows
@@ -103,14 +103,17 @@
             raise ValueError("a scalar vector is shorter than n")
     req.n, req.window_bits, req.scalars_mont, req.table, req.drop_zero_digits = n, window_bits, int(scalars_mont), int(table_c != 0), int(drop_zero_digits)
     req.c, req.row_first, req.row_step, req.sets, req.stride = table_c, row_first, row_step, sets, (stride if stride is not None else n)
-    req.by_rows, req.row_stride = int(rows > 0), (row_stride or 0)
+    req.by_rows, req.row_stride, req.spread = int(rows > 0), (row_stride or 0), int(bool(spread))
     for i, k in enumerate(keep[:3]):
         req.vec[i] = k.ctypes.data
     return keep
 
 
-def _msm_prep_plan(res) -> dict:
-    return dict({k: int(getattr(res, k)) for k in _lib.MSM_PREP_PLAN}, total=int(res.total), max_tasks=int(res.max_tasks))
+def _msm_prep_plan(res, spread=False) -> dict:
+    d = dict({k: int(getattr(res, k)) for k in _lib.MSM_PREP_PLAN}, total=int(res.total), max_tasks=int(res.max_tasks))
+    if spread:
+        d["spread_K"] = int(res.spread_K)
+    return d
 
 
 def _msm_prep_arrays(res, plan, arrays) -> dict:
@@ -125,18 +128,18 @@
 
 def msm_prep_inspect(vectors, n: int | None = None, window_bits: int = 0, scalars_mont: bool = False, table_c: int = 0, stride: int | None = None,
                      row_first: int = 0, row_step: int = 1, rows: int = 0, row_stride: int | None = None, drop_zero_digits: bool = False,
-                     plan_only: bool = False, arrays=None) -> dict:
+                     plan_only: bool = False, arrays=None, spread: bool = False) -> dict:
     req = _lib.MsmPrepRequest()
-    keep = _msm_prep_request(req, vectors, n, window_bits, scalars_mont, table_c, stride, row_first, row_step, rows, row_stride, drop_zero_digits)
+    keep = _msm_prep_request(req, vectors, n, window_bits, scalars_mont, table_c, stride, row_first, row_step, rows, row_stride, drop_zero_digits, spread)
     res = _lib.MsmPrepResult()
     check(lib().zk_bn254_msm_prep_inspect(C.byref(req), C.byref(res)))
-    out = _msm_prep_plan(res)
+    out = _msm_prep_plan(res, spread)
     if plan_only or out["total"] == 0:
         out.update(device_total=0, dropped=False, ctl=np.zeros(64, np.uint32), **{k: np.zeros(0, np.uint32) for k in _lib.MSM_PREP_ARRAYS})
         return out
     arrays = _msm_prep_arrays(res, out, arrays)
     check(lib().zk_bn254_msm_prep_inspect(C.byref(req), C.byref(res)))
-    assert _msm_prep_plan(res) == out
+    assert _msm_prep_plan(res, spread) == out
     out.update(device_total=int(res.device_total), dropped=bool(res.dropped), ctl=np.array(res.ctl[:], dtype=np.uint32), **arrays)
     return out
 
@@ -148,7 +151,7 @@
     req = _lib.MsmTailRequest()
     keep = _msm_prep_request(req.prep, vectors, prep.pop("n", None), prep.pop("window_bits", 0), prep.pop("scalars_mont", False), prep.pop("table_c", 0),
                              prep.pop("stride", None), prep.pop("row_first", 0), prep.pop("row_step", 1), prep.pop("rows", 0), prep.pop("row_stride", None),
-                             prep.pop("drop_zero_digits", False))
+                             prep.pop("drop_zero_digits", False), prep.pop("spread", False))
     if prep:
         raise TypeError("unknown arguments: %s" % sorted(prep))
     if pts.shape[0] < req.prep.n:
@@ -159,7 +162,7 @@
     check(lib().zk_bn254_msm_tail_inspect(C.byref(req), C.byref(res)))
 
     def plan():
-        d = _msm_prep_plan(res.prep)
+        d = _msm_prep_plan(res.prep, bool(req.prep.spread))
         d.update({k: int(getattr(res, k)) for k in ("m2", "n_final", "sh_final", "table_entries", "level_entries")})
         d["levels"] = [dict({k: int(getattr(res.level[i], k)) for k in _lib.MSM_TAIL_LEVEL}, kind=_lib.MSM_TAIL_KINDS[int(res.level[i].kind)])
                        for i in range(res.n_levels)]
diff --git a/noir_backend_using_gnark_amd/csrc/msm.hip b/noir_backend_using_gnark_amd/csrc/msm.hip
--- a/noir_backend_using_gnark_amd/csrc/msm.hip
+++ b/noir_backend_using_gnark_amd/csrc/msm.hip
@@ -112,9 +112,38 @@
     size_t stride;
     __device__ __forceinline__ const Fr* vec(unsigned v) const { return base + (size_t)v * stride; }
 };
+struct Scalar9 {
+    uint32_t l[9];
+};
+__device__ __forceinline__ Scalar9 spread_scalar(const Fr& s, uint32_t i, uint32_t K, unsigned c, unsigned W) {
+    Scalar9 t;
+#pragma unroll
+    for (int j = 0; j < 8; j++) t.l[j] = s.l[j];
+    t.l[8] = 0;
+    if (K <= 1) return t;
+    uint64_t bw = 0;
+#pragma unroll
+    for (int j = 0; j < 8; j++) bw = ((uint64_t)s.l[j] - FrParams::MOD[j] - bw) >> 63;
+    const unsigned shift = c * (W - 1), limb = shift >> 5, off = shift & 31;
+    uint32_t top = 0;
+#pragma unroll
+    for (unsigned j = 0; j < 8; j++) top |= j > limb ? s.l[j] : (j == limb ? s.l[j] >> off : 0u);
+    if (!bw || !top) return t;
+    const uint32_t k = i % K;
+    uint64_t acc = 0;
+#pragma unroll
+    for (int j = 0; j < 8; j++) {
+        acc += (uint64_t)k * FrParams::MOD[j] + s.l[j];
+        t.l[j] = (uint32_t)acc;
+        acc >>= 32;
+    }
+    t.l[8] = (uint32_t)acc;
+    return t;
+}
+
 template <class Src>
 __global__ void k_msm_digits(Src src, uint32_t n, int mont, unsigned c, unsigned W, uint32_t* keys, uint32_t* vals,
-                             uint32_t table_stride, unsigned row_first, unsigned row_step, unsigned rows_per_set) {
+                             uint32_t table_stride, unsigned row_first, unsigned row_step, unsigned rows_per_set, uint32_t spread_K) {
     prio_hi();
     uint32_t i = blockIdx.x * blockDim.x + threadIdx.x;
     if (i >= n) return;
@@ -128,6 +157,7 @@
         s.l[4] = b.x; s.l[5] = b.y; s.l[6] = b.z; s.l[7] = b.w;
     }
     if (mont) s = s.from_mont();
+    const Scalar9 t = spread_scalar(s, i, spread_K, c, W);
     const uint32_t B = 1u << (c - 1);
     const uint32_t sentinel = table_stride ? sets * B : W * B;
     uint32_t carry = 0;
@@ -135,9 +165,9 @@
     for (unsigned w = 0; w < W; w++) {
         unsigned bit = w * c, limb = bit >> 5, off = bit & 31;
         uint64_t v = 0;
-        if (limb < 8) {
-            v = s.l[limb];
-            if (limb + 1 < 8) v |= (uint64_t)s.l[limb + 1] << 32;
+        if (limb < 9) {
+            v = t.l[limb];
+            if (limb + 1 < 9) v |= (uint64_t)t.l[limb + 1] << 32;
             v >>= off;
         }
         uint32_t d = ((uint32_t)v & ((1u << c) - 1)) + carry;
@@ -172,16 +202,16 @@
     return mont ? s.from_mont() : s;
 }
 template <class Emit>
-__device__ __forceinline__ void digits_of(const Fr& s, unsigned c, unsigned W, bool table, unsigned row_first, unsigned row_step, Emit&& emit) {
+__device__ __forceinline__ void digits_of(const Scalar9& s, unsigned c, unsigned W, bool table, unsigned row_first, unsigned row_step, Emit&& emit) {
     const uint32_t B = 1u << (c - 1);
     uint32_t carry = 0;
     unsigned next_row = row_first, wl = 0;
     for (unsigned w = 0; w < W; w++) {
         unsigned bit = w * c, limb = bit >> 5, off = bit & 31;
         uint64_t v = 0;
-        if (limb < 8) {
+        if (limb < 9) {
             v = s.l[limb];
-            if (limb + 1 < 8) v |= (uint64_t)s.l[limb + 1] << 32;
+            if (limb + 1 < 9) v |= (uint64_t)s.l[limb + 1] << 32;
             v >>= off;
         }
         uint32_t d = ((uint32_t)v & ((1u << c) - 1)) + carry;
@@ -201,7 +231,8 @@
 }
 template <class Src>
 __global__ __launch_bounds__(256) void k_msm_digits_compact(Src src, uint32_t n, int mont, unsigned c, unsigned W, unsigned row_first, unsigned row_step,
-                                                           uint32_t table_stride, uint32_t* __restrict__ total, uint32_t* __restrict__ keys, uint32_t* __restrict__ vals) {
+                                                           uint32_t table_stride, uint32_t* __restrict__ total, uint32_t* __restrict__ keys, uint32_t* __restrict__ vals,
+                                                           uint32_t spread_K) {
     prio_hi();
     extern __shared__ uint32_t stage[];
     __shared__ uint32_t wsum[4];
@@ -211,9 +242,9 @@
     const uint32_t B = 1u << (c - 1), cap = 256u * W;
     const bool live = i < n;
     uint32_t k = 0;
-    Fr sc = Fr::zero();
+    Scalar9 sc = {};
     if (live) {
-        sc = canonical_scalar(src.vec(vec), i, mont);
+        sc = spread_scalar(canonical_scalar(src.vec(vec), i, mont), i, spread_K, c, W);
         digits_of(sc, c, W, table_stride != 0, row_first, row_step, [&](unsigned, uint32_t mag, uint32_t) { k += mag != 0; });
     }
     uint32_t incl = k;
@@ -852,32 +883,41 @@
     return best;
 }
 
+uint32_t msm_spread_K(unsigned c, unsigned Wd) {
+    static const uint32_t SPREAD_K[24] = {1, 2, 5, 10, 21, 42, 84, 169, 338, 677, 1354, 2708, 5417, 10834, 21668, 43336, 86673, 173347, 346695, 693390, 1386781, 2773562,
+                                          5547124, 11094248};
+    const unsigned e = c * Wd - 255;
+    return e < 24 ? SPREAD_K[e] : 1;
+}
+
 template <class F>
-static int msm_plan_uncached(size_t n, const zk_msm_cfg* cfg, hipStream_t st, MsmPlan* P, const MsmTable* tab, unsigned sets);
+static int msm_plan_uncached(size_t n, const zk_msm_cfg* cfg, hipStream_t st, MsmPlan* P, const MsmTable* tab, unsigned sets, bool spread);
 
 template <class F>
-static int msm_plan(size_t n, const zk_msm_cfg* cfg, hipStream_t st, MsmPlan* P, const MsmTable* tab = nullptr, unsigned sets = 1) {
+static int msm_plan(size_t n, const zk_msm_cfg* cfg, hipStream_t st, MsmPlan* P, const MsmTable* tab = nullptr, unsigned sets = 1, bool spread = true) {
     struct Key {
         size_t n, stride;
-        unsigned c_cfg, c_tab, g2, l1, rows, sets;
-        bool operator<(const Key& o) const { return std::tie(n, stride, c_cfg, c_tab, g2, l1, rows, sets) < std::tie(o.n, o.stride, o.c_cfg, o.c_tab, o.g2, o.l1, o.rows, o.sets); }
+        unsigned c_cfg, c_tab, g2, l1, rows, sets, spread;
+        bool operator<(const Key& o) const {
+            return std::tie(n, stride, c_cfg, c_tab, g2, l1, rows, sets, spread) < std::tie(o.n, o.stride, o.c_cfg, o.c_tab, o.g2, o.l1, o.rows, o.sets, o.spread);
+        }
     };
     static std::mutex mu;
     static std::map<Key, MsmPlan> memo;
-    Key k{n, tab ? tab->stride : 0, (cfg && cfg->window_bits) ? (unsigned)cfg->window_bits : 0u, tab ? tab->c : 0u, (unsigned)(sizeof(F) != 32), tab ? (tab->l1_m | (tab->l2_m << 8)) : 0u, tab ? (tab->row_first | (tab->row_step << 8)) : 0u, sets};
+    Key k{n, tab ? tab->stride : 0, (cfg && cfg->window_bits) ? (unsigned)cfg->window_bits : 0u, tab ? tab->c : 0u, (unsigned)(sizeof(F) != 32), tab ? (tab->l1_m | (tab->l2_m << 8)) : 0u, tab ? (tab->row_first | (tab->row_step << 8)) : 0u, sets, spread ? 1u : 0u};
     {
         std::lock_guard<std::mutex> lk(mu);
         auto it = memo.find(k);
         if (it != memo.end()) { *P = it->second; return ZK_OK; }
     }
-    ZK_TRY(msm_plan_uncached<F>(n, cfg, st, P, tab, sets));
+    ZK_TRY(msm_plan_uncached<F>(n, cfg, st, P, tab, sets, spread));
     std::lock_guard<std::mutex> lk(mu);
     memo[k] = *P;
     return ZK_OK;
 }
 
 template <class F>
-static int msm_plan_uncached(size_t n, const zk_msm_cfg* cfg, hipStream_t st, MsmPlan* P, const MsmTable* tab, unsigned sets) {
+static int msm_plan_uncached(size_t n, const zk_msm_cfg* cfg, hipStream_t st, MsmPlan* P, const MsmTable* tab, unsigned sets, bool spread) {
     typedef XYZZ<F> Pt;
     memset(P, 0, sizeof *P);
     if (n == 0) return ZK_OK;
@@ -893,6 +933,7 @@
     P->Wrows = tab ? tab->rows() : P->Wd;
     if (tab && P->Wrows == 0) { memset(P, 0, sizeof *P); return ZK_OK; }
     P->table_stride = tab ? (uint32_t)tab->stride : 0;
+    if (spread && tab && P->row_first == 0 && P->row_step == 1 && msm_spread_K(c, P->Wd) > 1) P->spread_K = msm_spread_K(c, P->Wd);
     P->B = 1u << (c - 1);
     if ((uint64_t)P->W << (c - 1) >= ((uint64_t)1 << 30)) return set_err(ZK_ERR_ARG, "%u bucket sets of 2^%u buckets overflow the sort keys", P->W, c - 1);
     P->nb = P->W * P->B;
@@ -900,7 +941,7 @@
     if (P->total >= ((size_t)1 << 31)) return set_err(ZK_ERR_ARG, "n * windows = %zu overflows 31-bit positions", P->total);
     if (tab && (size_t)tab->stride * P->Wrows >= ((size_t)1 << 31)) return set_err(ZK_ERR_ARG, "table too large for 31-bit indices");
     size_t mean = P->total / P->nb + 1;
-    {
+    if (P->spread_K <= 1) {
         const uint64_t r_top64 = 0x30644e72e131a029ULL;
         unsigned shift = c * (P->Wd - 1);
         uint64_t top_max = shift >= 192 ? (r_top64 >> (shift - 192)) : ~0ULL;
@@ -986,16 +1027,16 @@
             if (!cnt) return set_err(ZK_ERR_HIP, "MSM workspace was not reserved up front (zero-digit compaction)");
             ZK_HIP(hipMemsetAsync(cnt, 0, 4, st));
             if (rows) ZK_LAUNCH(s, st, "msm_digits", (k_msm_digits_compact<DigitRows>), grid, dim3(256), 256u * P.Wd * 8u, *rows, (uint32_t)n, mont, c, P.Wd, P.row_first, P.row_step,
-                                P.table_stride, cnt, keys0, vals0);
+                                P.table_stride, cnt, keys0, vals0, P.spread_K);
             else ZK_LAUNCH(s, st, "msm_digits", (k_msm_digits_compact<DigitSrc>), grid, dim3(256), 256u * P.Wd * 8u, src, (uint32_t)n, mont, c, P.Wd, P.row_first, P.row_step, P.table_stride, cnt,
-                           keys0, vals0);
+                           keys0, vals0, P.spread_K);
             d_total = cnt;
         } else if (rows) {
             ZK_LAUNCH(s, st, "msm_digits", (k_msm_digits<DigitRows>), grid, dim3(256), 0, *rows, (uint32_t)n, mont, c, P.Wd, keys0, vals0, P.table_stride, P.row_first, P.row_step,
-                      P.Wrows);
+                      P.Wrows, P.spread_K);
         } else {
             ZK_LAUNCH(s, st, "msm_digits", (k_msm_digits<DigitSrc>), grid, dim3(256), 0, src, (uint32_t)n, mont, c, P.Wd, keys0, vals0, P.table_stride, P.row_first, P.row_step,
-                      P.Wrows);
+                      P.Wrows, P.spread_K);
         }
     }
     PingPong kb(keys0, keys1), vb(vals0, vals1);
@@ -1411,10 +1452,10 @@
 }
 size_t msm_compact_need(size_t, unsigned) { return 1024; }
 int msm_prepare_scalars_table_batch(Slot* s, hipStream_t st, const void* const* d_scalars, unsigned sets, size_t n, const zk_msm_cfg* cfg, const MsmTable& tab, MsmPrep* out,
-                                    bool drop_zero_digits) {
+                                    bool drop_zero_digits, bool spread) {
     if (sets < 1 || sets > 3) return set_err(ZK_ERR_ARG, "a batch holds one to three scalar vectors");
     MsmPlan P;
-    ZK_TRY(msm_plan<Fp>(n, cfg, st, &P, &tab, sets));
+    ZK_TRY(msm_plan<Fp>(n, cfg, st, &P, &tab, sets, spread));
     DigitSrc src = {{nullptr, nullptr, nullptr}};
     for (unsigned v = 0; v < sets; v++) src.p[v] = (const Fr*)d_scalars[v];
     return msm_prepare(s, st, P, src.p[0], n, cfg, out, &src, drop_zero_digits);
@@ -1429,15 +1470,15 @@
     return ZK_OK;
 }
 int msm_prepare_scalars_table_rows(Slot* s, hipStream_t st, const void* d_base, size_t row_stride, unsigned sets, size_t n, const zk_msm_cfg* cfg, const MsmTable& tab,
-                                   MsmPrep* out, bool drop_zero_digits) {
+                                   MsmPrep* out, bool drop_zero_digits, bool spread) {
     MsmPlan P;
-    ZK_TRY(msm_plan<Fp>(n, cfg, st, &P, &tab, sets));
+    ZK_TRY(msm_plan<Fp>(n, cfg, st, &P, &tab, sets, spread));
     const DigitRows rows = {(const Fr*)d_base, row_stride};
     return msm_prepare(s, st, P, rows.base, n, cfg, out, nullptr, drop_zero_digits, &rows);
 }
-int msm_prepare_scalars_table(Slot* s, hipStream_t st, const void* d_scalars, size_t n, const zk_msm_cfg* cfg, const MsmTable& tab, MsmPrep* out, bool drop_zero_digits) {
+int msm_prepare_scalars_table(Slot* s, hipStream_t st, const void* d_scalars, size_t n, const zk_msm_cfg* cfg, const MsmTable& tab, MsmPrep* out, bool drop_zero_digits, bool spread) {
     MsmPlan P;
-    ZK_TRY(msm_plan<Fp>(n, cfg, st, &P, &tab));
+    ZK_TRY(msm_plan<Fp>(n, cfg, st, &P, &tab, 1, spread));
     return msm_prepare(s, st, P, (const Fr*)d_scalars, n, cfg, out, nullptr, drop_zero_digits);
 }
 
@@ -1759,9 +1800,9 @@
     }
     const bool drop = q->drop_zero_digits != 0;
     if (!tab) ZK_TRY(msm_prepare_scalars(s, st, d_vec[0], n, cfg, prep, drop));
-    else if (q->by_rows) ZK_TRY(msm_prepare_scalars_table_rows(s, st, d_vec[0], q->row_stride, sets, n, cfg, *tab, prep, drop));
-    else if (sets > 1) ZK_TRY(msm_prepare_scalars_table_batch(s, st, d_vec, sets, n, cfg, *tab, prep, drop));
-    else ZK_TRY(msm_prepare_scalars_table(s, st, d_vec[0], n, cfg, *tab, prep, drop));
+    else if (q->by_rows) ZK_TRY(msm_prepare_scalars_table_rows(s, st, d_vec[0], q->row_stride, sets, n, cfg, *tab, prep, drop, q->spread != 0));
+    else if (sets > 1) ZK_TRY(msm_prepare_scalars_table_batch(s, st, d_vec, sets, n, cfg, *tab, prep, drop, q->spread != 0));
+    else ZK_TRY(msm_prepare_scalars_table(s, st, d_vec[0], n, cfg, *tab, prep, drop, q->spread != 0));
     if (prep->empty && allow_empty && P.total == 0) return ZK_OK;
     if (prep->empty) return set_err(ZK_ERR_ARG, "MSM inspection: the preparation is empty where its plan is not");
     ZK_HIP(hipStreamSynchronize(st));
@@ -1800,7 +1841,8 @@
     } else if (q->sets > 1 || q->by_rows) {
         return set_err(ZK_ERR_ARG, "MSM inspection: several vectors need table mode");
     }
-    ZK_TRY(msm_plan<Fp>(q->n, cfg, nullptr, P, q->table ? tab : nullptr, q->table ? q->sets : 1));
+    ZK_TRY(msm_plan<Fp>(q->n, cfg, nullptr, P, q->table ? tab : nullptr, q->table ? q->sets : 1, q->spread != 0));
+    r->spread_K = P->spread_K;
     r->c = P->c; r->W = P->W; r->Wd = P->Wd; r->Wrows = P->Wrows; r->B = P->B; r->nb = P->nb; r->key_bits = P->key_bits; r->L = P->L; r->Lmin = P->Lmin;
     r->m1 = P->m1; r->N1 = P->N1; r->dropped = 0;
     r->total = P->total; r->max_tasks = P->max_tasks; r->device_total = 0;
@@ -1981,7 +2023,7 @@
     size_t need_acc = P.need_acc;
     if (q->is_g2) {
         MsmPlan P2;
-        ZK_TRY(msm_plan<Fp2>(pq->n, &cfg, nullptr, &P2, pq->table ? &tab : nullptr, pq->table ? pq->sets : 1));
+        ZK_TRY(msm_plan<Fp2>(pq->n, &cfg, nullptr, &P2, pq->table ? &tab : nullptr, pq->table ? pq->sets : 1, pq->spread != 0));
         need_acc = P2.need_acc;
     }
     r->m2 = P.m2;
diff --git a/noir_backend_using_gnark_amd/csrc/msm.hpp b/noir_backend_using_gnark_amd/csrc/msm.hpp
--- a/noir_backend_using_gnark_amd/csrc/msm.hpp
+++ b/noir_backend_using_gnark_amd/csrc/msm.hpp
@@ -39,6 +39,7 @@
     uint32_t table_stride;
     uint32_t B, nb, L, m1, N1, m2 = 0;
     uint32_t Lmin = 0;
+    uint32_t spread_K = 0;
     size_t total, max_tasks, sort_tmp_bytes, scan_tmp_bytes, tsort_tmp_bytes, lvl_elems, need, need_prep, need_acc;
 };
 struct MsmPrep {
@@ -87,14 +88,16 @@
 int msm_prep_need(size_t n, const zk_msm_cfg* cfg, hipStream_t st, size_t* need_prep, size_t* need_acc_g1, size_t* need_acc_g2);
 int msm_prepare_scalars(Slot* s, hipStream_t st, const void* d_scalars, size_t n, const zk_msm_cfg* cfg, MsmPrep* out, bool drop_zero_digits = false);
 int msm_prep_need_table(size_t n, const MsmTable& tab, hipStream_t st, size_t* need_prep, size_t* need_acc_g1, size_t* need_acc_g2);
-int msm_prepare_scalars_table(Slot* s, hipStream_t st, const void* d_scalars, size_t n, const zk_msm_cfg* cfg, const MsmTable& tab, MsmPrep* out, bool drop_zero_digits = false);
+uint32_t msm_spread_K(unsigned c, unsigned Wd);
+int msm_prepare_scalars_table(Slot* s, hipStream_t st, const void* d_scalars, size_t n, const zk_msm_cfg* cfg, const MsmTable& tab, MsmPrep* out, bool drop_zero_digits = false,
+                              bool spread = true);
 int msm_prep_need_table_batch(size_t n, unsigned sets, const MsmTable& tab, hipStream_t st, size_t* need_prep, size_t* need_acc_g1);
 int msm_prepare_scalars_table_batch(Slot* s, hipStream_t st, const void* const* d_scalars, unsigned sets, size_t n, const zk_msm_cfg* cfg, const MsmTable& tab, MsmPrep* out,
-                                    bool drop_zero_digits = false);
+                                    bool drop_zero_digits = false, bool spread = true);
 static constexpr unsigned MSM_MAX_SETS = 1024;
 int msm_prep_need_table_rows(size_t n, unsigned sets, const MsmTable& tab, hipStream_t st, size_t* need_prep, size_t* need_acc_g1, size_t* need_acc_g2);
 int msm_prepare_scalars_table_rows(Slot* s, hipStream_t st, const void* d_base, size_t row_stride, unsigned sets, size_t n, const zk_msm_cfg* cfg, const MsmTable& tab,
-                                   MsmPrep* out, bool drop_zero_digits = false);
+                                   MsmPrep* out, bool drop_zero_digits = false, bool spread = true);
 int msm_g1_finish_sets(const MsmJob& job, XYZZ<HFp>* out, unsigned sets);
 int msm_g2_finish_sets(const MsmJob& job, XYZZ<HFp2>* out, unsigned sets);
 size_t msm_compact_need(size_t n, unsigned sets);
```

Result: no change. 453.8 million G1 scalar-muls/s (whole prove: 4 G1 MSMs + G2 MSM + 7 NTTs per step), median of 6 (+0.7%).
